# chinokikiss/GSV-TTS-Lite

Measured on AMD Instinct MI355X. Metric: semantic_tokens_per_sec_end_to_end (GPT AR incl. prefill + flow/Generator vocoder); RTF^-1 = value/25, higher is better.
Workload: dtype bf16; 1 GPU; configs[1]: v2Pro bs=1 greedy AR decode (250 tokens, kv 200->450) + flow/Generator vocoder (500 frames = 10 s audio) per GPU per step, hipGraph on; parallelism=replicas x1, ge broadcast once per speaker (0 tensor broadcasts in this run)

## Files before the change

### gsv-tts-lite_amd/csrc/gsv_abi.hip

```cpp
#include <hip/hip_runtime.h>

#include <algorithm>
#include <cmath>
#include <cstddef>
#include <cstdlib>
#include <cstring>
#include <cstdint>
#include <map>
#include <mutex>
#include <type_traits>
#include <unordered_map>
#include <utility>
#include <vector>

namespace gsv_arena {
struct Arena {
    std::vector<std::pair<char*, size_t>> blocks;
    size_t used = 0;
    size_t count = 0;
    std::unordered_map<void*, size_t> live;
    std::multimap<size_t, void*> freed;
};
static std::mutex g_mu;
static std::vector<std::pair<std::pair<char*, size_t>, Arena*>> g_all;
static thread_local Arena* g_cur = nullptr;
static hipError_t amalloc(void** p, size_t n) {
    if (!g_cur) return hipMalloc(p, n);
    static const size_t align = getenv("GSV_ARENA_ALIGN") ? (size_t)atol(getenv("GSV_ARENA_ALIGN")) : 65536;
    static const size_t skew = getenv("GSV_ARENA_SKEW") ? (size_t)atol(getenv("GSV_ARENA_SKEW")) : 0;
    constexpr size_t kBlock = (size_t)256 << 20;
    Arena& a = *g_cur;
    bool reuse = false;
    {
        std::lock_guard<std::mutex> lk(g_mu);
        auto it = a.freed.lower_bound(n);
        if (it != a.freed.end() && it->first <= n + std::max<size_t>(n / 4, align)) {
            *p = it->second;
            a.live[*p] = it->first;
            a.freed.erase(it);
            reuse = true;
        }
    }
    if (reuse) {
        return hipDeviceSynchronize();
    }
    const size_t sk = (a.count * skew) % align;
    size_t start = (a.used + align - 1) / align * align + sk;
    if (a.blocks.empty() || start + n > a.blocks.back().second) {
        const size_t sz = std::max(n + align, kBlock);
        char* base = nullptr;
        const hipError_t e = hipMalloc(&base, sz);
        if (e != hipSuccess) return e;
        a.blocks.emplace_back(base, sz);
        a.used = 0;
        start = sk;
        std::lock_guard<std::mutex> lk(g_mu);
        g_all.push_back({{base, sz}, &a});
    }
    *p = a.blocks.back().first + start;
    a.used = start + n;
    a.count++;
    std::lock_guard<std::mutex> lk(g_mu);
    a.live[*p] = n;
    return hipSuccess;
}
static hipError_t afree(void* p) {
    {
        std::lock_guard<std::mutex> lk(g_mu);
        for (auto& b : g_all)
            if ((char*)p >= b.first.first && (char*)p < b.first.first + b.first.second) {
                Arena& a = *b.second;
                auto it = a.live.find(p);
                if (it != a.live.end()) {
                    a.freed.emplace(it->second, p);
                    a.live.erase(it);
                }
                return hipSuccess;
            }
    }
    return hipFree(p);
}
static void release(Arena& a) {
    std::lock_guard<std::mutex> lk(g_mu);
    for (auto& b : a.blocks) {
        (void)hipFree(b.first);
        g_all.erase(std::remove_if(g_all.begin(), g_all.end(), [&](const std::pair<std::pair<char*, size_t>, Arena*>& e) { return e.first == b; }),
                    g_all.end());
    }
    a.blocks.clear();
    a.live.clear();
    a.freed.clear();
    a.used = 0;
}
struct Scope {
    Arena* prev;
    explicit Scope(Arena* a) : prev(g_cur) { g_cur = a; }
    ~Scope() { g_cur = prev; }
};
}
#define GSV_DEV_ALLOC_ARENA 1

#include "abi_common.h"
#include "t2s_decode.h"
#include "t2s_decode_multi.h"
#include "t2s_batch.h"
#include "t2s_small.h"

namespace {
thread_local std::string g_err;
}

int gsv::abi_fail(int code, const char* fmt, ...) {
    char buf[512];
    va_list ap;
    va_start(ap, fmt);
    vsnprintf(buf, sizeof(buf), fmt, ap);
    va_end(ap);
    g_err = buf;
    return code;
}

struct T2SLayer {
    void *wqkv_p = nullptr, *wo_p = nullptr, *w1 = nullptr, *w2_p = nullptr;
    void* w2_p64 = nullptr;
    float *bqkv_p = nullptr, *bo = nullptr, *b1 = nullptr, *b2 = nullptr, *ln1g = nullptr, *ln1b = nullptr,
          *ln2g = nullptr, *ln2b = nullptr;
    PackedConv g_qkv, g_out, g_w1, g_w2;
    void *p8_qkv = nullptr, *p8_w1 = nullptr, *p8_w2 = nullptr;
    void *p16_qkv = nullptr, *p16_out = nullptr, *p16_w1 = nullptr, *p16_w2 = nullptr;
    void *f8_qkv = nullptr, *f8_w1 = nullptr, *f8_w2 = nullptr;
    float *s_qkv = nullptr, *s_w1 = nullptr, *s_w2 = nullptr;
    unsigned have = 0;
};

struct T2SStateX : gsv_t2s_state {
    int32_t* eos_host = nullptr;
    u32x4* tab = nullptr;
};
static_assert(sizeof(gsv_t2s_slot_sampling) == sizeof(u32x4) * kSlotSamplingWords, "the token kernel reads an entry as two 16-byte words");
inline u32x4* tab_of(const gsv_t2s_state& s) { return static_cast<const T2SStateX&>(s).tab; }
inline int32_t* eos_host_of(const gsv_t2s_state& s) { return static_cast<const T2SStateX&>(s).eos_host; }

struct T2SBound {
    T2SStateX st;
    hipGraphExec_t graph = nullptr;
    hipGraphExec_t graph_ft = nullptr;
    static constexpr int kMaxWin = 8;
    hipGraphExec_t wgraph[2][kMaxWin + 1] = {};
    int64_t *sg_kv = nullptr, *sg_x = nullptr;
    int32_t *sg_step = nullptr, *sg_eos = nullptr;
    float *sg_logits = nullptr, *sg_hidden = nullptr;
    TokPart* sg_tok = nullptr;
};

void t2s_drop_graphs(T2SBound& b) {
    if (b.graph) { (void)hipGraphExecDestroy(b.graph); b.graph = nullptr; }
    if (b.graph_ft) { (void)hipGraphExecDestroy(b.graph_ft); b.graph_ft = nullptr; }
    for (auto& row : b.wgraph)
        for (hipGraphExec_t& g : row)
            if (g) { (void)hipGraphExecDestroy(g); g = nullptr; }
}

void t2s_free_staging(T2SBound& b) {
    for (void* p : {(void*)b.sg_kv, (void*)b.sg_x, (void*)b.sg_step, (void*)b.sg_eos, (void*)b.sg_logits, (void*)b.sg_hidden, (void*)b.sg_tok})
        if (p) (void)gsv_dev_free(p);
    b.sg_kv = b.sg_x = nullptr; b.sg_step = b.sg_eos = nullptr; b.sg_logits = b.sg_hidden = nullptr; b.sg_tok = nullptr;
}

struct gsv_t2s {
    gsv_t2s_config cfg;
    std::vector<T2SLayer> layers;
    void* predict = nullptr;
    float *emb_audio = nullptr, *emb_text = nullptr, *pe_audio = nullptr, *pe_text = nullptr;
    PackedConv g_bert;
    unsigned have_io = 0;
    bool finalized = false;
    bool fp8 = false;
    int batched_min = 0;
    int nt_from_layer = 0x7fffffff;
    std::map<int, T2SBound> bound;
    int scratch_b = 0;
    float *xcur = nullptr, *xbuf = nullptr, *x1buf = nullptr, *ypart = nullptr, *zpart = nullptr;
    TokPart* tokpart = nullptr;
    hipStream_t cap_stream = nullptr;
    unsigned long long* dbg = nullptr;
    gsv_arena::Arena arena;
    bool use_arena = true;
};
#define GSV_ARENA_SCOPE(h) gsv_arena::Scope arena_scope_((h)->use_arena ? &(h)->arena : nullptr)

namespace {

int t2s_pack_fp8(const float* data, int cout, int cin, void** frag, float** scale, hipStream_t st) {
    const int mtiles = cdiv(cout, 32);
    if (!*scale) HIPCHK(gsv_dev_malloc(scale, sizeof(float) * mtiles * 32));
    if (!*frag) HIPCHK(gsv_dev_malloc(frag, (size_t)mtiles * (cin / 32) * 64 * 16));
    HIPCHK(hipMemsetAsync(*scale, 0, sizeof(float) * mtiles * 32, st));
    hipLaunchKernelGGL(fp8_row_scale_kernel, dim3(cdiv(cout, 4)), dim3(256), 0, st, data, cin, *scale, cout);
    hipLaunchKernelGGL(fp8_pack_kernel, dim3(1024), dim3(256), 0, st, data, (const float*)*scale, (uint32_t*)*frag, cout, cin, mtiles);
    HIPCHK(hipGetLastError());
    return GSV_OK;
}

int t2s_pack16_f8(void** dst, const float* data, const float* scale, int N, int K, hipStream_t st) {
    if (!*dst) HIPCHK(gsv_dev_malloc(dst, (size_t)N * K));
    hipLaunchKernelGGL(pack16_f8_kernel, dim3(1024), dim3(256), 0, st, data, scale, (uint32_t*)*dst, N, K);
    HIPCHK(hipGetLastError());
    return GSV_OK;
}

template <typename WT>
int t2s_pack16(void** dst, const float* data, int N, int K, hipStream_t st) {
    if (sizeof(WT) != 2) return GSV_OK;
    if (!*dst) HIPCHK(gsv_dev_malloc(dst, sizeof(bf16_t) * (size_t)N * K));
    hipLaunchKernelGGL(pack16_kernel, dim3(1024), dim3(256), 0, st, data, (bf16_t*)*dst, N, K);
    HIPCHK(hipGetLastError());
    return GSV_OK;
}

template <typename WT>
int t2s_load_layer_tensor(gsv_t2s* h, int l, const std::string& key, const float* data, int64_t numel, hipStream_t st) {
    T2SLayer& L = h->layers[l];
    auto want = [&](int64_t n) { return numel == n ? GSV_OK : fail(GSV_ERR_ARG, "layer %d %s: numel %lld, expected %lld", l, key.c_str(), (long long)numel, (long long)n); };
    auto copy_f32 = [&](float** dst, int64_t n, unsigned bit) -> int {
        if (int rc = want(n)) return rc;
        if (!*dst) HIPCHK(gsv_dev_malloc(dst, sizeof(float) * n));
        HIPCHK(hipMemcpyAsync(*dst, data, sizeof(float) * n, hipMemcpyDeviceToDevice, st));
        L.have |= bit;
        return GSV_OK;
    };
    if (key == "qkv.weight") {
        if (int rc = want(3LL * kD * kD)) return rc;
        if (!L.wqkv_p) HIPCHK(gsv_dev_malloc(&L.wqkv_p, sizeof(WT) * 3 * kD * kD));
        hipLaunchKernelGGL((pack_qkv_panel_kernel<WT>), dim3(1024), dim3(256), 0, st, data, (WT*)L.wqkv_p);
        float* keep = L.g_qkv.bias; L.g_qkv.bias = nullptr;
        free_conv(L.g_qkv);
        if (int rc = pack_conv<WT>(L.g_qkv, data, 3 * kD, kD, 1, kD, 1, 0, 1, 0, 0, nullptr, 1.f, st)) return rc;
        L.g_qkv.bias = keep;
        if (h->fp8) if (int rc = t2s_pack_fp8(data, 3 * kD, kD, &L.f8_qkv, &L.s_qkv, st)) return rc;
        if (h->fp8) if (int rc = t2s_pack16_f8(&L.p8_qkv, data, L.s_qkv, 3 * kD, kD, st)) return rc;
        if (int rc = t2s_pack16<WT>(&L.p16_qkv, data, 3 * kD, kD, st)) return rc;
        L.have |= 1u << 0;
    } else if (key == "qkv.bias") {
        if (int rc = want(3 * kD)) return rc;
        if (!L.bqkv_p) HIPCHK(gsv_dev_malloc(&L.bqkv_p, sizeof(float) * 3 * kD));
        hipLaunchKernelGGL(pack_qkv_bias_kernel, dim3(6), dim3(256), 0, st, data, L.bqkv_p);
        if (!L.g_qkv.bias) HIPCHK(gsv_dev_malloc(&L.g_qkv.bias, sizeof(float) * 3 * kD));
        HIPCHK(hipMemcpyAsync(L.g_qkv.bias, data, sizeof(float) * 3 * kD, hipMemcpyDeviceToDevice, st));
        L.have |= 1u << 1;
    } else if (key == "out_proj.weight") {
        if (int rc = want((int64_t)kD * kD)) return rc;
        if (!L.wo_p) HIPCHK(gsv_dev_malloc(&L.wo_p, sizeof(WT) * kD * kD));
        hipLaunchKernelGGL((pack_col_panel_kernel<WT>), dim3(512), dim3(256), 0, st, data, (WT*)L.wo_p, kH, kDh);
        free_conv(L.g_out);
        if (int rc = pack_conv<WT>(L.g_out, data, kD, kD, 1, kD, 1, 0, 1, 0, 0, nullptr, 1.f, st)) return rc;
        if (int rc = t2s_pack16<WT>(&L.p16_out, data, kD, kD, st)) return rc;
        L.have |= 1u << 2;
    } else if (key == "out_proj.bias") {
        if (int rc = copy_f32(&L.bo, kD, 1u << 3)) return rc;
    } else if (key == "mlp.0.weight") {
        if (int rc = want((int64_t)kF * kD)) return rc;
        if (!L.w1) HIPCHK(gsv_dev_malloc(&L.w1, sizeof(WT) * kF * kD));
        hipLaunchKernelGGL((convert_kernel<WT>), dim3(1024), dim3(256), 0, st, data, (WT*)L.w1, (size_t)kF * kD);
        free_conv(L.g_w1);
        if (int rc = pack_conv<WT>(L.g_w1, data, kF, kD, 1, kD, 1, 0, 1, 0, 0, nullptr, 1.f, st)) return rc;
        if (h->fp8) if (int rc = t2s_pack_fp8(data, kF, kD, &L.f8_w1, &L.s_w1, st)) return rc;
        if (h->fp8) if (int rc = t2s_pack16_f8(&L.p8_w1, data, L.s_w1, kF, kD, st)) return rc;
        if (int rc = t2s_pack16<WT>(&L.p16_w1, data, kF, kD, st)) return rc;
        L.have |= 1u << 4;
    } else if (key == "mlp.0.bias") {
        if (int rc = copy_f32(&L.b1, kF, 1u << 5)) return rc;
    } else if (key == "mlp.2.weight") {
        if (int rc = want((int64_t)kD * kF)) return rc;
        if (!L.w2_p) HIPCHK(gsv_dev_malloc(&L.w2_p, sizeof(WT) * kD * kF));
        hipLaunchKernelGGL((pack_col_panel_kernel<WT>), dim3(1024), dim3(256), 0, st, data, (WT*)L.w2_p, kNJ, kFJ);
        {
            if (!L.w2_p64) HIPCHK(gsv_dev_malloc(&L.w2_p64, sizeof(WT) * kD * kF));
            hipLaunchKernelGGL((pack_col_panel_kernel<WT>), dim3(1024), dim3(256), 0, st, data, (WT*)L.w2_p64, kNJFine, kF / kNJFine);
        }
        free_conv(L.g_w2);
        if (int rc = pack_conv<WT>(L.g_w2, data, kD, kF, 1, kF, 1, 0, 1, 0, 0, nullptr, 1.f, st)) return rc;
        if (h->fp8) if (int rc = t2s_pack_fp8(data, kD, kF, &L.f8_w2, &L.s_w2, st)) return rc;
        if (h->fp8) if (int rc = t2s_pack16_f8(&L.p8_w2, data, L.s_w2, kD, kF, st)) return rc;
        if (int rc = t2s_pack16<WT>(&L.p16_w2, data, kD, kF, st)) return rc;
        L.have |= 1u << 6;
    } else if (key == "mlp.2.bias") {
        if (int rc = copy_f32(&L.b2, kD, 1u << 7)) return rc;
    } else if (key == "norm1.weight") {
        if (int rc = copy_f32(&L.ln1g, kD, 1u << 8)) return rc;
    } else if (key == "norm1.bias") {
        if (int rc = copy_f32(&L.ln1b, kD, 1u << 9)) return rc;
    } else if (key == "norm2.weight") {
        if (int rc = copy_f32(&L.ln2g, kD, 1u << 10)) return rc;
    } else if (key == "norm2.bias") {
        if (int rc = copy_f32(&L.ln2b, kD, 1u << 11)) return rc;
    } else {
        return fail(GSV_ERR_ARG, "unknown layer tensor '%s'", key.c_str());
    }
    HIPCHK(hipGetLastError());
    return GSV_OK;
}

template <typename WT>
int t2s_load_io_tensor(gsv_t2s* h, const std::string& name, const float* data, int64_t numel, hipStream_t st) {
    const gsv_t2s_config& c = h->cfg;
    auto copy_f32 = [&](float** dst, int64_t n, unsigned bit) -> int {
        if (numel != n) return fail(GSV_ERR_ARG, "%s: numel %lld, expected %lld", name.c_str(), (long long)numel, (long long)n);
        if (!*dst) HIPCHK(gsv_dev_malloc(dst, sizeof(float) * n));
        HIPCHK(hipMemcpyAsync(*dst, data, sizeof(float) * n, hipMemcpyDeviceToDevice, st));
        h->have_io |= bit;
        return GSV_OK;
    };
    if (name == "ar_predict_layer.weight") {
        if (numel != (int64_t)c.vocab * kD) return fail(GSV_ERR_ARG, "%s: bad numel", name.c_str());
        if (!h->predict) HIPCHK(gsv_dev_malloc(&h->predict, sizeof(WT) * c.vocab * kD));
        hipLaunchKernelGGL((convert_kernel<WT>), dim3(512), dim3(256), 0, st, data, (WT*)h->predict, (size_t)c.vocab * kD);
        h->have_io |= 1u << 0;
    } else if (name == "ar_audio_embedding.word_embeddings.weight") {
        return copy_f32(&h->emb_audio, (int64_t)c.vocab * kD, 1u << 1);
    } else if (name == "ar_text_embedding.word_embeddings.weight") {
        return copy_f32(&h->emb_text, (int64_t)c.n_phoneme * kD, 1u << 2);
    } else if (name == "ar_audio_position.pe_scaled") {
        return copy_f32(&h->pe_audio, (int64_t)c.n_pos * kD, 1u << 3);
    } else if (name == "ar_text_position.pe_scaled") {
        return copy_f32(&h->pe_text, (int64_t)c.n_pos * kD, 1u << 4);
    } else if (name == "bert_proj.weight") {
        if (numel != (int64_t)kD * 1024) return fail(GSV_ERR_ARG, "%s: bad numel", name.c_str());
        float* keep = h->g_bert.bias; h->g_bert.bias = nullptr;
        free_conv(h->g_bert);
        if (int rc = pack_conv<WT>(h->g_bert, data, kD, 1024, 1, 1024, 1, 0, 1, 0, 0, nullptr, 1.f, st)) return rc;
        h->g_bert.bias = keep;
        h->have_io |= 1u << 5;
    } else if (name == "bert_proj.bias") {
        return copy_f32(&h->g_bert.bias, kD, 1u << 6);
    } else if (name == "ar_text_position.alpha" || name == "ar_audio_position.alpha") {
        return GSV_OK;
    } else {
        return fail(GSV_ERR_ARG, "unknown tensor '%s'", name.c_str());
    }
    HIPCHK(hipGetLastError());
    return GSV_OK;
}

int t2s_ensure_scratch(gsv_t2s* h, int B) {
    if (B <= h->scratch_b) return GSV_OK;
    for (void* p : {(void*)h->xcur, (void*)h->xbuf, (void*)h->x1buf, (void*)h->ypart, (void*)h->zpart, (void*)h->tokpart})
        if (p) (void)gsv_dev_free(p);
    HIPCHK(gsv_dev_malloc(&h->xcur, sizeof(float) * B * kD));
    HIPCHK(gsv_dev_malloc(&h->xbuf, sizeof(float) * B * kD));
    HIPCHK(gsv_dev_malloc(&h->x1buf, sizeof(float) * B * kD));
    HIPCHK(gsv_dev_malloc(&h->ypart, sizeof(float) * B * kH * kD));
    HIPCHK(gsv_dev_malloc(&h->zpart, sizeof(float) * B * kNJFine * kD));
    HIPCHK(gsv_dev_malloc(&h->tokpart, sizeof(TokPart) * B * kNP));
    HIPCHK(hipMemset(h->tokpart, 0, sizeof(TokPart) * B * kNP));
    h->scratch_b = B;
    for (auto& kv : h->bound) t2s_drop_graphs(kv.second);
    return GSV_OK;
}

template <typename WT>
void t2s_launch_attn(gsv_t2s* h, const gsv_t2s_state& s, int l, const float* xsrc, hipStream_t st, bool fused_token = false) {
    const int B = s.batch, T = s.max_kv;
    const size_t lds = 0;
    const size_t layer_elems = (size_t)B * kH * T * kDh;
    T2SLayer& L = h->layers[l];
    AttnArgs<WT> a;
    a.xdirect = xsrc;
    a.zpart = (const typename Geo<WT>::PT*)h->zpart;
    a.b2 = l ? h->layers[l - 1].b2 : nullptr;
    a.x1 = h->x1buf;
    a.ln2g = l ? h->layers[l - 1].ln2g : nullptr;
    a.ln2b = l ? h->layers[l - 1].ln2b : nullptr;
    a.xout = h->xbuf;
    a.wqkv = (const WT*)L.wqkv_p; a.bqkv = L.bqkv_p; a.wo = (const WT*)L.wo_p;
    a.kc = (WT*)s.k_cache + (size_t)l * layer_elems;
    a.vc = (WT*)s.v_cache + (size_t)l * layer_elems;
    a.kv_len = s.kv_len; a.T = T; a.ypart = (typename Geo<WT>::PT*)h->ypart; a.dbg = (l == h->cfg.n_layer - 1) ? h->dbg : nullptr;
    if (l == 0 && fused_token) {
        StepTok& k = a.tk;
        k.tokpart = h->tokpart; k.tok_override = s.tok_override; k.ctl = s.ctl; k.x_len = s.x_len; k.pre_tokens = s.pre_tokens;
        k.seen = s.seen; k.step = s.step; k.eos_at = s.eos_at; k.emb = h->emb_audio; k.pe = h->pe_audio; k.eos_host = eos_host_of(s);
        k.V = h->cfg.vocab; k.eos = h->cfg.eos; k.n_pos = h->cfg.n_pos;
    }
    auto with_mode = [&](auto launch) {
        if (l == 0 && fused_token) launch(std::integral_constant<int, 2>{});
        else if (l == 0) launch(std::integral_constant<int, 0>{});
        else launch(std::integral_constant<int, 1>{});
    };
    if (B > 16) {
        const size_t ml = sizeof(float) * attn_multi_lds_floats<2>();
        with_mode([&](auto mode) { hipLaunchKernelGGL((t2s_attn_multi_kernel<WT, decltype(mode)::value, 2>), dim3(kH, cdiv(B, 2)), dim3(kNT), ml, st, a, B); });
        return;
    }
    auto single = [&](auto nj, auto nt, auto ntkv) {
        with_mode([&](auto mode) {
            constexpr int MODE = decltype(mode)::value;
            constexpr int NJ = MODE == 1 ? decltype(nj)::value : kNJ;
            constexpr bool NT = MODE == 1 && decltype(nt)::value;
            hipLaunchKernelGGL((t2s_attn_kernel<WT, MODE, NJ, NT, decltype(ntkv)::value>), dim3(kH, B), dim3(kNT), lds, st, a);
        });
    };
    using Coarse = std::integral_constant<int, kNJ>;
    using Fine = std::integral_constant<int, kNJFine>;
    using NtF32 = std::bool_constant<sizeof(WT) == 4>;
    const bool fine = ffn_slices(B) == kNJFine;
    static const int kvnt_b = getenv("GSV_SEQ_KV_NT_MIN_B") ? atoi(getenv("GSV_SEQ_KV_NT_MIN_B")) : 4;
    if (sizeof(WT) == 2 && B >= kvnt_b) {
        if (fine) single(Fine{}, std::false_type{}, std::true_type{});
        else single(Coarse{}, std::false_type{}, std::true_type{});
        return;
    }
    const bool nt = sizeof(WT) == 4 && l >= h->nt_from_layer;
    if (fine && nt) single(Fine{}, NtF32{}, std::false_type{});
    else if (fine) single(Fine{}, std::false_type{}, std::false_type{});
    else if (nt) single(Coarse{}, NtF32{}, std::false_type{});
    else single(Coarse{}, std::false_type{}, std::false_type{});
}

template <typename WT>
void t2s_launch_ffn(gsv_t2s* h, const gsv_t2s_state& s, int l, hipStream_t st) {
    T2SLayer& L = h->layers[l];
    FfnArgs<WT> f;
    f.ypart = (const typename Geo<WT>::PT*)h->ypart; f.bo = L.bo; f.x = h->xbuf; f.ln1g = L.ln1g; f.ln1b = L.ln1b; f.x1out = h->x1buf;
    f.w1 = (const WT*)L.w1; f.b1 = L.b1; f.w2p = (const WT*)L.w2_p; f.zpart = (typename Geo<WT>::PT*)h->zpart; f.dbg = (l == h->cfg.n_layer - 1) ? h->dbg : nullptr;
    const int B = s.batch;
    static const int ffn_single_max_b = getenv("GSV_FFN_SINGLE_MAX_B") ? atoi(getenv("GSV_FFN_SINGLE_MAX_B")) : 8;
    if (B > ffn_single_max_b) {
        hipLaunchKernelGGL((t2s_ffn_multi_kernel<WT, 2>), dim3(kNJ, cdiv(B, 2)), dim3(kNT), sizeof(float) * ffn_multi_lds_floats<2>(), st, f, B);
        return;
    }
    auto single = [&](auto nj) {
        constexpr int NJ = decltype(nj)::value;
        if (sizeof(WT) == 4 && l >= h->nt_from_layer) hipLaunchKernelGGL((t2s_ffn_kernel<WT, NJ, sizeof(WT) == 4>), dim3(NJ, B), dim3(kNT), 0, st, f);
        else hipLaunchKernelGGL((t2s_ffn_kernel<WT, NJ>), dim3(NJ, B), dim3(kNT), 0, st, f);
    };
    if (ffn_slices(B) == kNJFine) {
        f.w2p = (const WT*)L.w2_p64;
        single(std::integral_constant<int, kNJFine>{});
    } else {
        single(std::integral_constant<int, kNJ>{});
    }
}

template <typename WT>
int t2s_multi_lds_attr() {
    const int la = (int)(sizeof(float) * attn_multi_lds_floats<2>());
    HIPCHK(hipFuncSetAttribute((const void*)t2s_attn_multi_kernel<WT, 0, 2>, hipFuncAttributeMaxDynamicSharedMemorySize, la));
    HIPCHK(hipFuncSetAttribute((const void*)t2s_attn_multi_kernel<WT, 1, 2>, hipFuncAttributeMaxDynamicSharedMemorySize, la));
    HIPCHK(hipFuncSetAttribute((const void*)t2s_attn_multi_kernel<WT, 2, 2>, hipFuncAttributeMaxDynamicSharedMemorySize, la));
    HIPCHK(hipFuncSetAttribute((const void*)t2s_ffn_multi_kernel<WT, 2>, hipFuncAttributeMaxDynamicSharedMemorySize, (int)(sizeof(float) * ffn_multi_lds_floats<2>())));
    return GSV_OK;
}

template <typename WT>
int t2s_layers(gsv_t2s* h, const gsv_t2s_state& s, const float* xsrc, hipStream_t st, bool fused_token = false) {
    for (int l = 0; l < h->cfg.n_layer; ++l) {
        t2s_launch_attn<WT>(h, s, l, xsrc, st, fused_token);
        t2s_launch_ffn<WT>(h, s, l, st);
    }
    HIPCHK(hipGetLastError());
    return GSV_OK;
}

template <typename WT>
int t2s_logits(gsv_t2s* h, const gsv_t2s_state& s, int mode, const float* hdirect, int slot0, int nrows, int vlimit,
               int bump, hipStream_t st, const int32_t* slots = nullptr, const T2SBound* staged = nullptr) {
    const T2SLayer& L = h->layers.back();
    LogitsArgs<WT> a;
    a.hdirect = hdirect; a.zpart = (const typename Geo<WT>::PT*)h->zpart; a.b2 = L.b2; a.x1 = h->x1buf; a.ln2g = L.ln2g; a.ln2b = L.ln2b;
    a.wp = (const WT*)h->predict; a.V = h->cfg.vocab; a.eos = h->cfg.eos; a.vlimit = vlimit; a.slot0 = slot0; a.slots = slots;
    a.step = s.step; a.ctl = s.ctl; a.fctl = s.fctl; a.seen = s.seen; a.logits = s.logits; a.hidden = s.hidden;
    a.tokpart = h->tokpart; a.kv_len = s.kv_len; a.bump = bump;
    if (staged) { a.step = staged->sg_step; a.logits = staged->sg_logits; a.hidden = staged->sg_hidden; a.tokpart = staged->sg_tok; a.kv_len = staged->sg_kv; }
    a.tab = tab_of(s);
    auto launch = [&](auto tab) {
        constexpr bool TAB = decltype(tab)::value;
        if (mode == 0) hipLaunchKernelGGL((t2s_logits_kernel<WT, 0, kNJ, TAB>), dim3(kNP, nrows), dim3(kNT), 0, st, a);
        else if (ffn_slices(s.batch) == kNJFine) hipLaunchKernelGGL((t2s_logits_kernel<WT, 1, kNJFine, TAB>), dim3(kNP, nrows), dim3(kNT), 0, st, a);
        else hipLaunchKernelGGL((t2s_logits_kernel<WT, 1, kNJ, TAB>), dim3(kNP, nrows), dim3(kNT), 0, st, a);
    };
    if (a.tab) launch(std::true_type{});
    else launch(std::false_type{});
    HIPCHK(hipGetLastError());
    return GSV_OK;
}

int t2s_token(gsv_t2s* h, const gsv_t2s_state& s, int advance, hipStream_t st) {
    TokenArgs a;
    a.tokpart = h->tokpart; a.tok_override = s.tok_override; a.ctl = s.ctl; a.kv_len = s.kv_len; a.x_len = s.x_len;
    a.pre_tokens = s.pre_tokens; a.seen = s.seen; a.step = s.step; a.eos_at = s.eos_at; a.eos_host = eos_host_of(s); a.emb = h->emb_audio;
    a.pe = h->pe_audio; a.xcur = h->xcur; a.T = s.max_kv; a.V = h->cfg.vocab; a.eos = h->cfg.eos; a.n_pos = h->cfg.n_pos;
    a.advance = advance;
    a.logits = s.logits; a.fctl = s.fctl; a.tab = tab_of(s);
    if (a.tab) hipLaunchKernelGGL(t2s_token_kernel<true>, dim3(s.batch), dim3(256), 0, st, a);
    else hipLaunchKernelGGL(t2s_token_kernel<false>, dim3(s.batch), dim3(256), 0, st, a);
    HIPCHK(hipGetLastError());
    return GSV_OK;
}

constexpr int kBatchedMinDefault = 17;
constexpr int kWideMinM = 3072;
constexpr size_t kPrefillLdsMax = 160 * 1024;
constexpr int kNtFromLayerF32 = 9;

struct ChainBufs {
    float *qkv, *attn, *y1, *y2, *x1;
    void* hid;
};

template <typename AttnFn>
int t2s_gemm_chain(gsv_t2s* h, int M, float* x0, const ChainBufs& c, bool f8, AttnFn attn_launch, hipStream_t st, bool prompt = false) {
    const int rtiles = cdiv(M, 32);
    const int cpb = !prompt ? 1 : (rtiles < 40 ? 2 : (rtiles < 100 ? 4 : 8));
    auto run = [&](auto kern, int nthreads, BGemmArgs ba, int which = -1) {
        int cb = cpb;
        if (prompt && which >= 0) {
            if (rtiles <= 20 && (which == 1 || which == 3)) cb = 1;
            if (rtiles > 20 && rtiles < 40 && (which == 0 || which == 2)) cb = 4;
        }
        ba.cpb = cb;
        hipLaunchKernelGGL(kern, dim3(rtiles, cdiv(ba.mtiles, cb)), dim3(nthreads), 0, st, ba);
    };
    static const int small_max = getenv("GSV_SMALL_MAX_M") ? atoi(getenv("GSV_SMALL_MAX_M")) : kSmallMaxM;
    const bool small = !prompt && M <= small_max && h->layers[0].p16_qkv != nullptr && (!f8 || h->layers[0].p8_qkv != nullptr);
    const int rt16 = cdiv(M, 16);
    const bool nwv4 = M > 48;
    static const int wide_min = getenv("GSV_WIDE_MIN_M") ? atoi(getenv("GSV_WIDE_MIN_M")) : kWideMinM;
    const bool wide = prompt && !f8 && M >= wide_min;
    auto run_wide = [&](auto kern, bool w2, BGemmArgs ba) -> int {
        const int rgroups = cdiv(M, 32 * kWideRT), cgroups = cdiv(ba.mtiles, 4 * kWideTPW);
        int gpb = 1;
        if (!w2) {
            double best = 1e30;
            for (int g = 1; g <= cgroups; ++g) {
                if (cgroups % g) continue;
                const double cost = (double)cdiv(rgroups * (cgroups / g), 256) * (1.0 + g);
                if (cost < best - 1e-9) { best = cost; gpb = g; }
            }
        }
        ba.cpb = gpb * 4 * kWideTPW;
        hipLaunchKernelGGL(kern, dim3(rgroups, cgroups / gpb), dim3(256), kWideLds, st, ba);
        return GSV_OK;
    };
    for (int l = 0; l < h->cfg.n_layer; ++l) {
        T2SLayer& L = h->layers[l];
        if (wide) {
            {
                BGemmArgs g{};
                g.M = M; g.ldx = kD; g.W = (const uint4*)L.g_qkv.w; g.mtiles = 3 * kD / 32; g.cout = 3 * kD; g.bias = L.g_qkv.bias; g.Y = c.qkv; g.ldy = 3 * kD;
                if (l == 0) {
                    g.X = x0;
                    if (int rc = run_wide(bgemm_wide_kernel<PRO_NONE, float, bf16_t>, false, g)) return rc;
                } else {
                    g.X = c.y2; g.lng = h->layers[l - 1].ln2g; g.lnb = h->layers[l - 1].ln2b; g.xout = x0;
                    if (int rc = run_wide(bgemm_wide_kernel<PRO_LN, float, bf16_t>, false, g)) return rc;
                }
            }
            attn_launch(l);
            {
                BGemmArgs g{};
                g.M = M; g.X = c.attn; g.ldx = kD; g.W = (const uint4*)L.g_out.w; g.mtiles = kD / 32; g.cout = kD; g.bias = L.bo;
                g.res = x0; g.ldres = kD; g.Y = c.y1; g.ldy = kD;
                if (int rc = run_wide(bgemm_wide_kernel<PRO_NONE, bf16_t, float>, false, g)) return rc;
            }
            {
                BGemmArgs g{};
                g.M = M; g.X = c.y1; g.ldx = kD; g.lng = L.ln1g; g.lnb = L.ln1b; g.xout = c.x1;
                g.W = (const uint4*)L.g_w1.w; g.mtiles = kF / 32; g.cout = kF; g.bias = L.b1; g.relu = 1; g.Y = c.hid; g.ldy = kF;
                if (int rc = run_wide(bgemm_wide_kernel<PRO_LN, float, bf16_t>, false, g)) return rc;
            }
            {
                BGemmArgs g{};
                g.M = M; g.X = c.hid; g.ldx = kF; g.W = (const uint4*)L.g_w2.w; g.mtiles = kD / 32; g.cout = kD;
                g.bias = L.b2; g.res = c.x1; g.ldres = kD; g.Y = c.y2; g.ldy = kD;
                if (int rc = run_wide(bgemm_wide_kernel<PRO_NONE, bf16_t, float>, true, g)) return rc;
            }
            continue;
        }
        if (small) {
            {
                SGemmArgs g{};
                g.M = M; g.W = (const uint4*)(f8 ? L.p8_qkv : L.p16_qkv); g.wscale = L.s_qkv; g.bias = L.g_qkv.bias; g.Y = c.qkv; g.ldy = 3 * kD;
                const dim3 grid(rt16, 3 * kD / 32);
                if (l == 0) {
                    g.X = x0;
                    if (f8) hipLaunchKernelGGL((sgemm_kernel<PRO_NONE, float, 2, true>), grid, dim3(128), 0, st, g);
                    else hipLaunchKernelGGL((sgemm_kernel<PRO_NONE, float, 2>), grid, dim3(128), 0, st, g);
                } else {
                    g.X = c.y2; g.lng = h->layers[l - 1].ln2g; g.lnb = h->layers[l - 1].ln2b; g.xout = x0;
                    const dim3 grid4(rt16, 3 * kD / 64);
                    if (f8 && nwv4) hipLaunchKernelGGL((sgemm_kernel<PRO_LN, float, 4, true>), grid4, dim3(256), 0, st, g);
                    else if (f8) hipLaunchKernelGGL((sgemm_kernel<PRO_LN, float, 2, true>), grid, dim3(128), 0, st, g);
                    else if (nwv4) hipLaunchKernelGGL((sgemm_kernel<PRO_LN, float, 4>), grid4, dim3(256), 0, st, g);
                    else hipLaunchKernelGGL((sgemm_kernel<PRO_LN, float, 2>), grid, dim3(128), 0, st, g);
                }
            }
            attn_launch(l);
            {
                SGemmArgs g{};
                g.M = M; g.X = c.attn; g.W = (const uint4*)L.p16_out; g.bias = L.bo; g.res = x0; g.Y = c.y1; g.ldy = kD;
                hipLaunchKernelGGL((sgemm_kernel<PRO_NONE, float, 2>), dim3(rt16, kD / 32), dim3(128), 0, st, g);
            }
            {
                SGemmArgs g{};
                g.M = M; g.X = c.y1; g.lng = L.ln1g; g.lnb = L.ln1b; g.xout = c.x1; g.W = (const uint4*)(f8 ? L.p8_w1 : L.p16_w1); g.wscale = L.s_w1;
                g.bias = L.b1; g.relu = 1; g.Y = c.hid; g.ldy = kF;
                if (f8 && nwv4) hipLaunchKernelGGL((sgemm_kernel<PRO_LN, fp8_t, 4, true>), dim3(rt16, kF / 64), dim3(256), 0, st, g);
                else if (f8) hipLaunchKernelGGL((sgemm_kernel<PRO_LN, fp8_t, 2, true>), dim3(rt16, kF / 32), dim3(128), 0, st, g);
                else if (nwv4) hipLaunchKernelGGL((sgemm_kernel<PRO_LN, bf16_t, 4>), dim3(rt16, kF / 64), dim3(256), 0, st, g);
                else hipLaunchKernelGGL((sgemm_kernel<PRO_LN, bf16_t, 2>), dim3(rt16, kF / 32), dim3(128), 0, st, g);
            }
            {
                SGemmArgs g{};
                g.M = M; g.X = c.hid; g.W = (const uint4*)(f8 ? L.p8_w2 : L.p16_w2); g.wscale = L.s_w2; g.bias = L.b2; g.res = c.x1; g.Y = c.y2; g.ldy = kD;
                if (f8) hipLaunchKernelGGL(sgemm_k_kernel<true>, dim3(rt16, kD / 16), dim3(256), 0, st, g);
                else hipLaunchKernelGGL(sgemm_k_kernel<false>, dim3(rt16, kD / 16), dim3(256), 0, st, g);
            }
            continue;
        }
        {
            BGemmArgs g{};
            g.M = M; g.ldx = kD; g.W = (const uint4*)(f8 ? L.f8_qkv : L.g_qkv.w); g.wscale = L.s_qkv; g.mtiles = 3 * kD / 32; g.cout = 3 * kD;
            g.bias = L.g_qkv.bias; g.Y = c.qkv; g.ldy = 3 * kD;
            if (l == 0) {
                g.X = x0;
                if (f8) run(bgemm_kernel<PRO_NONE, float, float, 4, true>, 256, g);
                else if (prompt) run(bgemm_kernel<PRO_NONE, float, bf16_t, 4, false, true>, 256, g, 0);
                else run(bgemm_kernel<PRO_NONE, float, float, 4, false, true>, 256, g);
            } else {
                g.X = c.y2; g.lng = h->layers[l - 1].ln2g; g.lnb = h->layers[l - 1].ln2b; g.xout = x0;
                if (f8) run(bgemm_kernel<PRO_LN, float, float, 4, true>, 256, g);
                else if (prompt) run(bgemm_kernel<PRO_LN, float, bf16_t, 4, false, true>, 256, g, 0);
                else run(bgemm_kernel<PRO_LN, float, float, 4, false, true>, 256, g);
            }
        }
        attn_launch(l);
        {
            BGemmArgs g{};
            g.M = M; g.X = c.attn; g.ldx = kD; g.W = (const uint4*)L.g_out.w; g.mtiles = kD / 32; g.cout = kD; g.bias = L.bo;
            g.res = x0; g.ldres = kD; g.Y = c.y1; g.ldy = kD;
            if (prompt) run(bgemm_kernel<PRO_NONE, bf16_t, float, 4, false>, 256, g, 1);
            else run(bgemm_kernel<PRO_NONE, float, float, 4, false, true>, 256, g);
        }
        {
            BGemmArgs g{};
            g.M = M; g.X = c.y1; g.ldx = kD; g.lng = L.ln1g; g.lnb = L.ln1b; g.xout = c.x1;
            g.W = (const uint4*)(f8 ? L.f8_w1 : L.g_w1.w); g.wscale = L.s_w1; g.mtiles = kF / 32; g.cout = kF; g.bias = L.b1; g.relu = 1;
            g.Y = c.hid; g.ldy = kF;
            if (f8) run(bgemm_kernel<PRO_LN, float, fp8_t, 4, true>, 256, g);
            else run(bgemm_kernel<PRO_LN, float, bf16_t, 4, false, true>, 256, g, 2);
        }
        {
            BGemmArgs g{};
            g.M = M; g.X = c.hid; g.ldx = kF; g.W = (const uint4*)(f8 ? L.f8_w2 : L.g_w2.w); g.wscale = L.s_w2; g.mtiles = kD / 32; g.cout = kD;
            g.bias = L.b2; g.res = c.x1; g.ldres = kD; g.Y = c.y2; g.ldy = kD;
            if (f8) run(bgemm_kernel<PRO_NONE, fp8_t, float, 16, true>, 1024, g);
            else run(bgemm_kernel<PRO_NONE, bf16_t, float, 16, false>, 1024, g, 3);
        }
    }
    HIPCHK(hipGetLastError());
    return GSV_OK;
}

template <typename WT>
int t2s_batched_layers(gsv_t2s* h, const gsv_t2s_state& s, hipStream_t st) {
    const int B = s.batch, T = s.max_kv;
    ChainBufs c;
    c.qkv = h->ypart;
    c.attn = c.qkv + (size_t)B * 3 * kD;
    c.y1 = c.attn + (size_t)B * kD;
    c.y2 = c.y1 + (size_t)B * kD;
    c.x1 = h->x1buf;
    c.hid = h->zpart;
    const size_t layer_elems = (size_t)B * kH * T * kDh;
    auto attn = [&](int l) {
        BatchAttnArgs<WT> ba;
        ba.qkv = c.qkv; ba.kc = (WT*)s.k_cache + (size_t)l * layer_elems; ba.vc = (WT*)s.v_cache + (size_t)l * layer_elems;
        ba.kv_len = s.kv_len; ba.T = T; ba.out = c.attn; ba.dbg = (l == h->cfg.n_layer - 1) ? h->dbg : nullptr;
        if (T <= 256) hipLaunchKernelGGL((t2s_batch_attn2_kernel<4, true>), dim3(kH, B), dim3(256), 0, st, ba);
        else if (T <= 512) hipLaunchKernelGGL((t2s_batch_attn2_kernel<8, true>), dim3(kH, B), dim3(256), 0, st, ba);
        else hipLaunchKernelGGL((t2s_batch_attn2_kernel<16, true>), dim3(kH, B), dim3(256), 0, st, ba);
    };
    if (int rc = t2s_gemm_chain(h, B, h->xcur, c, h->fp8, attn, st)) return rc;
    const T2SLayer& LL = h->layers.back();
    hipLaunchKernelGGL(ln_rows_kernel, dim3(cdiv(B, 4)), dim3(256), 0, st, (const float*)c.y2, (const float*)LL.ln2g, (const float*)LL.ln2b, h->xbuf, B);
    HIPCHK(hipGetLastError());
    return GSV_OK;
}

template <typename WT>
int t2s_step(gsv_t2s* h, const gsv_t2s_state& s, hipStream_t st, bool fused_token = false) {
    if (fused_token && !(sizeof(WT) == 2 && s.batch >= h->batched_min && s.max_kv <= 1024)) {
        if (int rc = t2s_layers<WT>(h, s, h->xcur, st, true)) return rc;
        return t2s_logits<WT>(h, s, 1, nullptr, 0, s.batch, h->cfg.vocab, 1, st);
    }
    if (int rc = t2s_token(h, s, 1, st)) return rc;
    if constexpr (sizeof(WT) == 2) {
        if (s.batch >= h->batched_min && s.max_kv <= 1024) {
            if (int rc = t2s_batched_layers<WT>(h, s, st)) return rc;
            return t2s_logits<WT>(h, s, 0, h->xbuf, 0, s.batch, h->cfg.vocab, 1, st);
        }
    }
    if (int rc = t2s_layers<WT>(h, s, h->xcur, st)) return rc;
    return t2s_logits<WT>(h, s, 1, nullptr, 0, s.batch, h->cfg.vocab, 1, st);
}

template <typename WT>
int t2s_prefill_impl(gsv_t2s* h, T2SBound& bd, int slot0, int nrows, int l_max, float* xy, const int64_t* x_lens,
                     const int64_t* y_lens, void* ws, size_t ws_bytes, hipStream_t st, const int32_t* slots = nullptr, bool staged = false) {
    const gsv_t2s_state& s = bd.st;
    const int M = nrows * l_max, T = s.max_kv;
    const size_t need = gsv_t2s_prefill_workspace(h, nrows, l_max);
    if (ws_bytes < need) return fail(GSV_ERR_ARG, "prefill workspace %zu < %zu", ws_bytes, need);
    float* qkv = (float*)ws;
    float* attn = qkv + (size_t)M * 3 * kD;
    float* ybuf = attn + (size_t)M * kD;
    float* fbuf = ybuf + (size_t)M * kD;
    float* hlast = fbuf + (size_t)M * kF;
    const size_t layer_elems = (size_t)s.batch * kH * T * kDh;
    const int qsplit = std::max(1, std::min(16, 256 / (kH * nrows)));
    const size_t lds = sizeof(float) * ((size_t)l_max * 33 + (size_t)l_max * 32 + 4 * (size_t)l_max + 128 + 8);
    const int nkt_max = cdiv(l_max, 32);
    const size_t lds_mfma = (size_t)nkt_max * 32 * 80 + 128 * 80 + (size_t)32 * (nkt_max * 64 + 16);
    if (sizeof(WT) == 2 ? lds_mfma > kPrefillLdsMax : lds > kPrefillLdsMax)
        return fail(GSV_ERR_ARG, "prefill: prompt of %d positions exceeds the LDS-staged attention limit of the %s mode (%d positions)",
                    l_max, sizeof(WT) == 2 ? "bf16" : "fp32", sizeof(WT) == 2 ? 1056 : 591);
    if constexpr (sizeof(WT) == 2) {
        ChainBufs c;
        c.qkv = qkv; c.attn = attn; c.y1 = ybuf; c.y2 = fbuf; c.x1 = fbuf + (size_t)M * kD; c.hid = fbuf + (size_t)2 * M * kD;
        auto attn_launch = [&](int l) {
            PrefillAttnMfmaArgs pm;
            pm.qkv = (const bf16_t*)qkv; pm.x_lens = x_lens; pm.y_lens = y_lens;
            pm.kc = (bf16_t*)s.k_cache + (size_t)l * layer_elems; pm.vc = (bf16_t*)s.v_cache + (size_t)l * layer_elems;
            pm.T = T; pm.slot0 = slot0; pm.slots = slots; pm.l_max = l_max; pm.out = (bf16_t*)attn;
            hipLaunchKernelGGL(t2s_prefill_attn_mfma_kernel, dim3(kH, nrows, cdiv(l_max, 128)), dim3(256), lds_mfma, st, pm);
        };
        if (int rc = t2s_gemm_chain(h, M, xy, c, false, attn_launch, st, true)) return rc;
        const T2SLayer& LL = h->layers.back();
        hipLaunchKernelGGL(ln_rows_kernel, dim3(cdiv(M, 4)), dim3(256), 0, st, (const float*)c.y2, (const float*)LL.ln2g, (const float*)LL.ln2b, xy, M);
        HIPCHK(hipGetLastError());
    } else {
        for (int l = 0; l < h->cfg.n_layer; ++l) {
            T2SLayer& L = h->layers[l];
            Epi e0; e0.fixed_order = true;
            if (int rc = run_conv<float, WT, float>(L.g_qkv, xy, kD, M, qkv, 3 * kD, M, e0, st)) return rc;
            PrefillAttnArgs<WT> pa;
            pa.qkv = qkv; pa.x_lens = x_lens; pa.y_lens = y_lens;
            pa.kc = (WT*)s.k_cache + (size_t)l * layer_elems; pa.vc = (WT*)s.v_cache + (size_t)l * layer_elems;
            pa.T = T; pa.slot0 = slot0; pa.slots = slots; pa.l_max = l_max; pa.qsplit = qsplit; pa.out = attn;
            {
                hipLaunchKernelGGL((t2s_prefill_attn_kernel<WT>), dim3(kH, nrows, qsplit), dim3(256), lds, st, pa);
            }
            Epi e1; e1.res = xy; e1.ld_res = kD; e1.fixed_order = true;
            PackedConv go = L.g_out; go.bias = L.bo;
            if (int rc = run_conv<float, WT, float>(go, attn, kD, M, ybuf, kD, M, e1, st)) return rc;
            hipLaunchKernelGGL(ln_rows_kernel, dim3(cdiv(M, 4)), dim3(256), 0, st, ybuf, L.ln1g, L.ln1b, xy, M);
            Epi e2; e2.act = ACT_RELU; e2.fixed_order = true;
            PackedConv g1 = L.g_w1; g1.bias = L.b1;
            if (int rc = run_conv<float, WT, float>(g1, xy, kD, M, fbuf, kF, M, e2, st)) return rc;
            Epi e3; e3.res = xy; e3.ld_res = kD; e3.fixed_order = true;
            PackedConv g2 = L.g_w2; g2.bias = L.b2;
            if (int rc = run_conv<float, WT, float>(g2, fbuf, kF, M, ybuf, kD, M, e3, st)) return rc;
            hipLaunchKernelGGL(ln_rows_kernel, dim3(cdiv(M, 4)), dim3(256), 0, st, ybuf, L.ln2g, L.ln2b, xy, M);
        }
    }
    PrefillFinishArgs fa;
    fa.hidden = xy; fa.x_lens = x_lens; fa.y_lens = y_lens; fa.hlast = hlast; fa.kv_len = s.kv_len; fa.x_len = s.x_len;
    fa.step = s.step; fa.eos_at = s.eos_at; fa.eos_host = bd.st.eos_host; fa.slot0 = slot0; fa.slots = slots; fa.l_max = l_max;
    if (staged) { fa.kv_len = bd.sg_kv; fa.x_len = bd.sg_x; fa.step = bd.sg_step; fa.eos_at = bd.sg_eos; fa.eos_host = nullptr; }
    hipLaunchKernelGGL(t2s_prefill_finish_kernel, dim3(nrows), dim3(128), 0, st, fa);
    HIPCHK(hipGetLastError());
    return t2s_logits<WT>(h, s, 0, hlast, slot0, nrows, h->cfg.vocab - 1, 0, st, slots, staged ? &bd : nullptr);
}

struct CommitArgs {
    const int32_t* slots;
    const int64_t *sg_kv, *sg_x; const int32_t *sg_step, *sg_eos; const float *sg_logits, *sg_hidden; const TokPart* sg_tok;
    int64_t *kv_len, *x_len; int32_t *step, *eos_at, *eos_host; float *logits, *hidden; TokPart* tokpart;
    int V;
};
__global__ __launch_bounds__(256) void t2s_commit_kernel(CommitArgs a) {
    const int s = a.slots[blockIdx.x], tid = threadIdx.x;
    for (int v = tid; v < a.V; v += 256) a.logits[(size_t)s * a.V + v] = a.sg_logits[(size_t)s * a.V + v];
    for (int c = tid; c < kD; c += 256) a.hidden[(size_t)s * kD + c] = a.sg_hidden[(size_t)s * kD + c];
    if (tid < kNP) a.tokpart[(size_t)s * kNP + tid] = a.sg_tok[(size_t)s * kNP + tid];
    if (tid == 0) { a.kv_len[s] = a.sg_kv[s]; a.x_len[s] = a.sg_x[s]; a.step[s] = a.sg_step[s]; a.eos_at[s] = a.sg_eos[s]; eos_publish(a.eos_host, s, a.sg_eos[s]); }
}


constexpr int kAdoptMax = 64;
struct AdoptArgs {
    short dst[kAdoptMax], src[kAdoptMax];
    long long ovr[kAdoptMax];
    const unsigned char *ks, *vs;
    unsigned char *kd, *vd;
    int Bs, Ts, Bd, Td, esz;
    const int64_t *sg_kv, *sg_x; const int32_t *sg_step, *sg_eos; const float *sg_logits, *sg_hidden; const TokPart* sg_tok;
    int64_t *kv_len, *x_len, *tok_override; int32_t *step, *eos_at, *eos_host; float *logits, *hidden; TokPart* tokpart;
    const unsigned char* s_seen; unsigned char* d_seen;
    int V;
};
__global__ __launch_bounds__(256) void t2s_adopt_kv_kernel(AdoptArgs a) {
    const int lh = blockIdx.x, r = blockIdx.y, l = lh / kH, hd = lh % kH;
    const int ss = a.src[r], ds = a.dst[r];
    long long kv = a.sg_kv[ss];
    kv = kv < 0 ? 0 : (kv > a.Ts ? a.Ts : kv);
    kv = kv > a.Td ? a.Td : kv;
    const size_t n16 = (size_t)kv * kDh * a.esz / 16;
    const size_t so = ((((size_t)l * a.Bs + ss) * kH + hd) * a.Ts) * kDh * a.esz;
    const size_t d0 = ((((size_t)l * a.Bd + ds) * kH + hd) * a.Td) * kDh * a.esz;
    const uint4* sp = reinterpret_cast<const uint4*>((blockIdx.z ? a.vs : a.ks) + so);
    uint4* dp = reinterpret_cast<uint4*>((blockIdx.z ? a.vd : a.kd) + d0);
    for (size_t i = threadIdx.x; i < n16; i += 256) dp[i] = sp[i];
}
__global__ __launch_bounds__(256) void t2s_adopt_state_kernel(AdoptArgs a) {
    const int ss = a.src[blockIdx.x], s = a.dst[blockIdx.x], tid = threadIdx.x;
    for (int v = tid; v < a.V; v += 256) { a.logits[(size_t)s * a.V + v] = a.sg_logits[(size_t)ss * a.V + v]; a.d_seen[(size_t)s * a.V + v] = a.s_seen[(size_t)ss * a.V + v]; }
    for (int c = tid; c < kD; c += 256) a.hidden[(size_t)s * kD + c] = a.sg_hidden[(size_t)ss * kD + c];
    if (tid < kNP) a.tokpart[(size_t)s * kNP + tid] = a.sg_tok[(size_t)ss * kNP + tid];
    if (tid == 0) {
        a.kv_len[s] = a.sg_kv[ss]; a.x_len[s] = a.sg_x[ss]; a.step[s] = a.sg_step[ss]; a.eos_at[s] = a.sg_eos[ss];
        eos_publish(a.eos_host, s, a.sg_eos[ss]);
        if (a.ovr[blockIdx.x] >= 0) a.tok_override[s] = a.ovr[blockIdx.x];
    }
}

struct MoveArgs {
    short dst[kAdoptMax], src[kAdoptMax];
    const unsigned char *ks, *vs; unsigned char *kd, *vd;
    int Bs, Ts, Bd, Td, esz, V, n;
    const int64_t *s_kv, *s_x, *s_pre, *s_ovr; const int32_t *s_step, *s_eos; const float *s_logits, *s_hidden; const unsigned char* s_seen;
    int64_t *d_kv, *d_x, *d_pre, *d_ovr; int32_t *d_step, *d_eos, *d_eos_host; float *d_logits, *d_hidden; unsigned char* d_seen;
    TokPart* tokpart;
    const u32x4* s_tab; u32x4* d_tab;
};
__global__ __launch_bounds__(256) void t2s_move_kv_kernel(MoveArgs a) {
    const int lh = blockIdx.x, r = blockIdx.y, l = lh / kH, hd = lh % kH;
    const int ss = a.src[r], ds = a.dst[r];
    long long kv = a.s_kv[ss];
    kv = kv < 0 ? 0 : (kv > a.Ts ? a.Ts : kv);
    kv = kv > a.Td ? a.Td : kv;
    const size_t n16 = (size_t)kv * kDh * a.esz / 16;
    const size_t so = ((((size_t)l * a.Bs + ss) * kH + hd) * a.Ts) * kDh * a.esz;
    const size_t d0 = ((((size_t)l * a.Bd + ds) * kH + hd) * a.Td) * kDh * a.esz;
    const uint4* sp = reinterpret_cast<const uint4*>((blockIdx.z ? a.vs : a.ks) + so);
    uint4* dp = reinterpret_cast<uint4*>((blockIdx.z ? a.vd : a.kd) + d0);
    for (size_t i = threadIdx.x; i < n16; i += 256) dp[i] = sp[i];
}
__global__ __launch_bounds__(256) void t2s_move_state_kernel(MoveArgs a) {
    const int tid = threadIdx.x;
    if (blockIdx.x == a.n) {
        __shared__ TokPart tp[kAdoptMax * kNP];
        for (int i = tid; i < a.n * kNP; i += 256) tp[i] = a.tokpart[(size_t)a.src[i / kNP] * kNP + i % kNP];
        __syncthreads();
        for (int i = tid; i < a.n * kNP; i += 256) a.tokpart[(size_t)a.dst[i / kNP] * kNP + i % kNP] = tp[i];
        return;
    }
    const int ss = a.src[blockIdx.x], s = a.dst[blockIdx.x];
    for (int v = tid; v < a.V; v += 256) { a.d_logits[(size_t)s * a.V + v] = a.s_logits[(size_t)ss * a.V + v]; a.d_seen[(size_t)s * a.V + v] = a.s_seen[(size_t)ss * a.V + v]; }
    for (int c = tid; c < kD; c += 256) a.d_hidden[(size_t)s * kD + c] = a.s_hidden[(size_t)ss * kD + c];
    const int np = (a.Ts < a.Td ? a.Ts : a.Td) + 1;
    for (int t = tid; t < np; t += 256) a.d_pre[(size_t)s * (a.Td + 1) + t] = a.s_pre[(size_t)ss * (a.Ts + 1) + t];
    if (tid == 0) {
        a.d_kv[s] = a.s_kv[ss]; a.d_x[s] = a.s_x[ss]; a.d_step[s] = a.s_step[ss]; a.d_eos[s] = a.s_eos[ss]; a.d_ovr[s] = a.s_ovr[ss];
        eos_publish(a.d_eos_host, s, a.s_eos[ss]);
    }
    if (a.s_tab != nullptr && tid < kSlotSamplingWords) a.d_tab[kSlotSamplingWords * s + tid] = a.s_tab[kSlotSamplingWords * ss + tid];
}

struct PutSamplingArgs {
    short slot[kAdoptMax];
    u32x4 e[kAdoptMax][kSlotSamplingWords];
    u32x4* tab;
};
__global__ __launch_bounds__(64) void t2s_put_sampling_kernel(PutSamplingArgs a) {
    const int r = blockIdx.x, tid = threadIdx.x;
    if (tid < kSlotSamplingWords) a.tab[kSlotSamplingWords * a.slot[r] + tid] = a.e[r][tid];
}

struct SeedSeenArgs {
    short slot[kAdoptMax];
    int off[kAdoptMax + 1];
    const int64_t* tokens;
    unsigned char* seen;
    int V;
};
__global__ __launch_bounds__(256) void t2s_seed_seen_kernel(SeedSeenArgs a) {
    const int r = blockIdx.x, tid = threadIdx.x;
    unsigned char* row = a.seen + (size_t)a.slot[r] * a.V;
    for (int v = tid; v < a.V; v += 256) row[v] = 0;
    __syncthreads();
    for (int i = a.off[r] + tid; i < a.off[r + 1]; i += 256) {
        const int64_t t = a.tokens[i];
        if (t >= 0 && t < a.V) row[t] = 1;
    }
}

}

template <typename WT>
static int t2s_time_impl(gsv_t2s* h, T2SBound* b, int iters, float* out_ms, hipStream_t st) {
    struct Guard {
        hipEvent_t e0 = nullptr, e1 = nullptr;
        hipGraphExec_t exec = nullptr;
        ~Guard() {
            if (exec) (void)hipGraphExecDestroy(exec);
            if (e0) (void)hipEventDestroy(e0);
            if (e1) (void)hipEventDestroy(e1);
        }
    } gd;
    HIPCHK(hipEventCreate(&gd.e0));
    HIPCHK(hipEventCreate(&gd.e1));
    const int NL = h->cfg.n_layer;
    for (int cls = 0; cls < 4; ++cls) {
        hipGraph_t g = nullptr;
        HIPCHK(hipStreamSynchronize(st));
        HIPCHK(hipStreamBeginCapture(h->cap_stream, hipStreamCaptureModeThreadLocal));
        int rc = GSV_OK;
        for (int l = 0; l < NL && !rc; ++l) {
            if (cls == 0) t2s_launch_attn<WT>(h, b->st, l, h->xcur, h->cap_stream);
            if (cls == 1) t2s_launch_ffn<WT>(h, b->st, l, h->cap_stream);
            if (cls == 2) rc = t2s_logits<WT>(h, b->st, 1, nullptr, 0, b->st.batch, h->cfg.vocab, 0, h->cap_stream);
            if (cls == 3) rc = t2s_token(h, b->st, 0, h->cap_stream);
        }
        hipError_t e = hipStreamEndCapture(h->cap_stream, &g);
        if (rc) { if (g) (void)hipGraphDestroy(g); return rc; }
        if (e != hipSuccess) return fail(GSV_ERR_HIP, "hipStreamEndCapture: %s", hipGetErrorString(e));
        e = hipGraphInstantiate(&gd.exec, g, nullptr, nullptr, 0);
        (void)hipGraphDestroy(g);
        if (e != hipSuccess) { gd.exec = nullptr; return fail(GSV_ERR_HIP, "hipGraphInstantiate: %s", hipGetErrorString(e)); }
        HIPCHK(hipGraphLaunch(gd.exec, st));
        HIPCHK(hipEventRecord(gd.e0, st));
        for (int it = 0; it < iters; ++it) HIPCHK(hipGraphLaunch(gd.exec, st));
        HIPCHK(hipEventRecord(gd.e1, st));
        HIPCHK(hipEventSynchronize(gd.e1));
        float ms = 0.f;
        HIPCHK(hipEventElapsedTime(&ms, gd.e0, gd.e1));
        out_ms[cls] = ms / (float)(iters * NL);
        (void)hipGraphExecDestroy(gd.exec);
        gd.exec = nullptr;
    }
    return GSV_OK;
}

extern "C" {

int gsv_version(void) { return 1; }
const char* gsv_last_error(void) { return g_err.c_str(); }

int gsv_t2s_create(const gsv_t2s_config* cfg, gsv_t2s** out) {
    if (!cfg || !out) return fail(GSV_ERR_ARG, "null argument");
    if (cfg->hidden != kD || cfg->n_head != kH)
        return fail(GSV_ERR_ARG, "unsupported GPT shape: hidden %d heads %d (kernels are specialised for 512/16)", cfg->hidden, cfg->n_head);
    if (cfg->vocab < 2 || cfg->vocab > kNP * 128 || cfg->n_layer < 1 || cfg->n_pos < 1)
        return fail(GSV_ERR_ARG, "unsupported vocab/n_layer/n_pos");
    if (cfg->dtype != GSV_F32 && cfg->dtype != GSV_BF16 && cfg->dtype != GSV_FP8) return fail(GSV_ERR_ARG, "bad dtype");
    gsv_t2s* h = new gsv_t2s();
    h->cfg = *cfg;
    if (cfg->dtype == GSV_FP8) { h->fp8 = true; h->cfg.dtype = GSV_BF16; }
    h->batched_min = kBatchedMinDefault;
    if (const char* e = getenv("GSV_BATCHED_MIN")) h->batched_min = std::max(1, atoi(e));
    if (h->cfg.dtype == GSV_F32) h->nt_from_layer = kNtFromLayerF32;
    if (const char* e = getenv("GSV_NT_FROM_LAYER")) h->nt_from_layer = atoi(e);
    if (getenv("GSV_NO_ARENA")) h->use_arena = false;
    h->layers.resize(cfg->n_layer);
    if (hipStreamCreateWithFlags(&h->cap_stream, hipStreamNonBlocking) != hipSuccess) {
        delete h;
        return fail(GSV_ERR_HIP, "hipStreamCreate failed");
    }
    *out = h;
    return GSV_OK;
}

int gsv_t2s_destroy(gsv_t2s* h) {
    if (!h) return GSV_OK;
    (void)hipDeviceSynchronize();
    for (auto& kv : h->bound) {
        t2s_drop_graphs(kv.second);
        t2s_free_staging(kv.second);
    }
    for (T2SLayer& L : h->layers) {
        for (void* p : {L.wqkv_p, L.wo_p, L.w1, L.w2_p, L.w2_p64, L.p16_qkv, L.p16_out, L.p16_w1, L.p16_w2, L.p8_qkv, L.p8_w1, L.p8_w2, (void*)L.bqkv_p, (void*)L.bo, (void*)L.b1, (void*)L.b2,
                        (void*)L.ln1g, (void*)L.ln1b, (void*)L.ln2g, (void*)L.ln2b, L.f8_qkv, L.f8_w1, L.f8_w2,
                        (void*)L.s_qkv, (void*)L.s_w1, (void*)L.s_w2})
            if (p) (void)gsv_dev_free(p);
        free_conv(L.g_qkv); L.g_out.bias = nullptr; free_conv(L.g_out); L.g_w1.bias = nullptr; free_conv(L.g_w1);
        L.g_w2.bias = nullptr; free_conv(L.g_w2);
    }
    for (void* p : {h->predict, (void*)h->emb_audio, (void*)h->emb_text, (void*)h->pe_audio, (void*)h->pe_text,
                    (void*)h->xcur, (void*)h->xbuf, (void*)h->x1buf, (void*)h->ypart, (void*)h->zpart, (void*)h->tokpart})
        if (p) (void)gsv_dev_free(p);
    free_conv(h->g_bert);
    if (h->cap_stream) (void)hipStreamDestroy(h->cap_stream);
    gsv_arena::release(h->arena);
    delete h;
    return GSV_OK;
}

int gsv_t2s_load_tensor(gsv_t2s* h, const char* name, const float* data, int64_t numel, void* stream) {
    if (!h || !name || !data) return fail(GSV_ERR_ARG, "null argument");
    GSV_ARENA_SCOPE(h);
    std::string n(name);
    const std::string pre = "t2s_transformer.blocks.";
    h->finalized = false;
    if (n.compare(0, pre.size(), pre) == 0) {
        size_t dot = n.find('.', pre.size());
        if (dot == std::string::npos) return fail(GSV_ERR_ARG, "bad tensor name '%s'", name);
        int l = atoi(n.substr(pre.size(), dot - pre.size()).c_str());
        if (l < 0 || l >= h->cfg.n_layer) return fail(GSV_ERR_ARG, "layer index out of range in '%s'", name);
        std::string key = n.substr(dot + 1);
        return h->cfg.dtype == GSV_BF16 ? t2s_load_layer_tensor<bf16_t>(h, l, key, data, numel, S(stream))
                                        : t2s_load_layer_tensor<float>(h, l, key, data, numel, S(stream));
    }
    return h->cfg.dtype == GSV_BF16 ? t2s_load_io_tensor<bf16_t>(h, n, data, numel, S(stream))
                                    : t2s_load_io_tensor<float>(h, n, data, numel, S(stream));
}

int gsv_t2s_finalize(gsv_t2s* h, void* stream) {
    if (!h) return fail(GSV_ERR_ARG, "null handle");
    GSV_ARENA_SCOPE(h);
    for (int l = 0; l < h->cfg.n_layer; ++l)
        if (h->layers[l].have != 0xfffu) return fail(GSV_ERR_STATE, "layer %d incomplete (mask 0x%x)", l, h->layers[l].have);
    if (h->have_io != 0x7fu) return fail(GSV_ERR_STATE, "embedding/predict tensors incomplete (mask 0x%x)", h->have_io);
    if (h->cfg.dtype == GSV_BF16) {
        HIPCHK(hipFuncSetAttribute((const void*)t2s_prefill_attn_mfma_kernel, hipFuncAttributeMaxDynamicSharedMemorySize, (int)kPrefillLdsMax));
        HIPCHK(hipFuncSetAttribute((const void*)bgemm_wide_kernel<PRO_NONE, float, bf16_t>, hipFuncAttributeMaxDynamicSharedMemorySize, (int)kWideLds));
        HIPCHK(hipFuncSetAttribute((const void*)bgemm_wide_kernel<PRO_LN, float, bf16_t>, hipFuncAttributeMaxDynamicSharedMemorySize, (int)kWideLds));
        HIPCHK(hipFuncSetAttribute((const void*)bgemm_wide_kernel<PRO_NONE, bf16_t, float>, hipFuncAttributeMaxDynamicSharedMemorySize, (int)kWideLds));
        if (int rc = t2s_multi_lds_attr<bf16_t>()) return rc;
    } else {
        HIPCHK(hipFuncSetAttribute((const void*)t2s_prefill_attn_kernel<float>, hipFuncAttributeMaxDynamicSharedMemorySize, (int)kPrefillLdsMax));
        if (int rc = t2s_multi_lds_attr<float>()) return rc;
    }
    HIPCHK(hipStreamSynchronize(S(stream)));
    h->finalized = true;
    return GSV_OK;
}

int gsv_t2s_bind_state(gsv_t2s* h, const gsv_t2s_state* st) {
    if (!h || !st) return fail(GSV_ERR_ARG, "null argument");
    GSV_ARENA_SCOPE(h);
    if (st->batch < 1 || st->max_kv < 2) return fail(GSV_ERR_ARG, "bad batch/max_kv");
    if (!st->k_cache || !st->v_cache || !st->kv_len || !st->x_len || !st->pre_tokens || !st->seen || !st->step ||
        !st->eos_at || !st->logits || !st->hidden || !st->tok_override || !st->ctl || !st->fctl)
        return fail(GSV_ERR_ARG, "state has null pointers");
    if (int rc = t2s_ensure_scratch(h, st->batch)) return rc;
    T2SBound& b = h->bound[st->batch];
    t2s_drop_graphs(b);
    static_cast<gsv_t2s_state&>(b.st) = *st;
    b.st.eos_host = nullptr;
    b.st.tab = nullptr;
    t2s_free_staging(b);
    const size_t B = (size_t)st->batch;
    HIPCHK(gsv_dev_malloc(&b.sg_kv, 8 * B)); HIPCHK(gsv_dev_malloc(&b.sg_x, 8 * B));
    HIPCHK(gsv_dev_malloc(&b.sg_step, 4 * B)); HIPCHK(gsv_dev_malloc(&b.sg_eos, 4 * B));
    HIPCHK(gsv_dev_malloc(&b.sg_logits, sizeof(float) * B * h->cfg.vocab)); HIPCHK(gsv_dev_malloc(&b.sg_hidden, sizeof(float) * B * kD));
    HIPCHK(gsv_dev_malloc(&b.sg_tok, sizeof(TokPart) * B * kNP));
    HIPCHK(hipMemset(b.sg_step, 0, 4 * B));
    HIPCHK(hipMemset(b.sg_kv, 0, 8 * B)); HIPCHK(hipMemset(b.sg_x, 0, 8 * B));
    HIPCHK(hipMemset(b.sg_eos, 0xff, 4 * B));
    return GSV_OK;
}

int gsv_t2s_unbind_state(gsv_t2s* h, int batch) {
    if (!h) return fail(GSV_ERR_ARG, "null handle");
    GSV_ARENA_SCOPE(h);
    auto it = h->bound.find(batch);
    if (it == h->bound.end()) return GSV_OK;
    T2SBound& b = it->second;
    t2s_drop_graphs(b);
    t2s_free_staging(b);
    h->bound.erase(it);
    return GSV_OK;
}

static T2SBound* t2s_find(gsv_t2s* h, int batch) {
    auto it = h->bound.find(batch);
    return it == h->bound.end() ? nullptr : &it->second;
}

int gsv_t2s_embed_prompt(gsv_t2s* h, int nrows, int lx_max, int ly_max, int l_max, const int64_t* x_ids,
                         const int64_t* y_ids, const float* bert, const int64_t* x_lens, const int64_t* y_lens,
                         float* xy, float* scratch, void* stream) {
    if (!h || !h->finalized) return fail(GSV_ERR_STATE, "handle not finalized");
    if (nrows < 1 || lx_max < 1 || ly_max < 1 || l_max < 1 || l_max > h->cfg.n_pos) return fail(GSV_ERR_ARG, "bad sizes");
    const int M = nrows * lx_max;
    Epi e;
    e.fixed_order = true;
    int rc = h->cfg.dtype == GSV_BF16 ? run_conv<float, bf16_t, float>(h->g_bert, bert, 1024, M, scratch, kD, M, e, S(stream))
                                      : run_conv<float, float, float>(h->g_bert, bert, 1024, M, scratch, kD, M, e, S(stream));
    if (rc) return rc;
    EmbedArgs a;
    a.x_ids = x_ids; a.y_ids = y_ids; a.proj = scratch; a.x_lens = x_lens; a.y_lens = y_lens; a.emb_text = h->emb_text;
    a.emb_audio = h->emb_audio; a.pe_text = h->pe_text; a.pe_audio = h->pe_audio; a.xy = xy; a.lx_max = lx_max;
    a.ly_max = ly_max; a.l_max = l_max; a.n_phoneme = h->cfg.n_phoneme; a.V = h->cfg.vocab;
    hipLaunchKernelGGL(t2s_embed_kernel, dim3(l_max, nrows), dim3(128), 0, S(stream), a);
    HIPCHK(hipGetLastError());
    return GSV_OK;
}

size_t gsv_t2s_prefill_workspace(gsv_t2s* h, int nrows, int l_max) {
    (void)h;
    const size_t M = (size_t)nrows * l_max;
    return sizeof(float) * (M * (3 * kD + kD + kD + kF) + (size_t)nrows * kD) + 256;
}

int gsv_t2s_prefill(gsv_t2s* h, int batch, int slot0, int nrows, int l_max, float* xy, const int64_t* x_lens,
                    const int64_t* y_lens, void* workspace, size_t workspace_bytes, void* stream) {
    if (!h || !h->finalized) return fail(GSV_ERR_STATE, "handle not finalized");
    T2SBound* b = t2s_find(h, batch);
    if (!b) return fail(GSV_ERR_STATE, "no state bound for batch %d", batch);
    if (slot0 < 0 || nrows < 1 || slot0 + nrows > batch) return fail(GSV_ERR_ARG, "slot range out of bounds");
    if (l_max < 1 || l_max > b->st.max_kv) return fail(GSV_ERR_ARG, "prompt of %d positions does not fit the KV cache (%d)", l_max, b->st.max_kv);
    return h->cfg.dtype == GSV_BF16
               ? t2s_prefill_impl<bf16_t>(h, *b, slot0, nrows, l_max, xy, x_lens, y_lens, workspace, workspace_bytes, S(stream))
               : t2s_prefill_impl<float>(h, *b, slot0, nrows, l_max, xy, x_lens, y_lens, workspace, workspace_bytes, S(stream));
}

int gsv_t2s_prefill_slots(gsv_t2s* h, int batch, const int32_t* slots, int nrows, int l_max, float* xy, const int64_t* x_lens,
                          const int64_t* y_lens, void* workspace, size_t workspace_bytes, void* stream) {
    if (!h || !h->finalized) return fail(GSV_ERR_STATE, "handle not finalized");
    T2SBound* b = t2s_find(h, batch);
    if (!b) return fail(GSV_ERR_STATE, "no state bound for batch %d", batch);
    if (!slots || nrows < 1 || nrows > batch) return fail(GSV_ERR_ARG, "prefill_slots: need 1..batch rows and their slot list");
    if (l_max < 1 || l_max > b->st.max_kv) return fail(GSV_ERR_ARG, "prompt of %d positions does not fit the KV cache (%d)", l_max, b->st.max_kv);
    return h->cfg.dtype == GSV_BF16
               ? t2s_prefill_impl<bf16_t>(h, *b, 0, nrows, l_max, xy, x_lens, y_lens, workspace, workspace_bytes, S(stream), slots)
               : t2s_prefill_impl<float>(h, *b, 0, nrows, l_max, xy, x_lens, y_lens, workspace, workspace_bytes, S(stream), slots);
}

int gsv_t2s_prefill_slots_staged(gsv_t2s* h, int batch, const int32_t* slots, int nrows, int l_max, float* xy, const int64_t* x_lens,
                                 const int64_t* y_lens, void* workspace, size_t workspace_bytes, void* stream) {
    if (!h || !h->finalized) return fail(GSV_ERR_STATE, "handle not finalized");
    T2SBound* b = t2s_find(h, batch);
    if (!b) return fail(GSV_ERR_STATE, "no state bound for batch %d", batch);
    if (!slots || nrows < 1 || nrows > batch) return fail(GSV_ERR_ARG, "prefill_slots_staged: need 1..batch rows and their slot list");
    if (l_max < 1 || l_max > b->st.max_kv - 1) return fail(GSV_ERR_ARG, "prompt of %d positions does not fit beside the parking row of the KV cache (%d)", l_max, b->st.max_kv);
    return h->cfg.dtype == GSV_BF16
               ? t2s_prefill_impl<bf16_t>(h, *b, 0, nrows, l_max, xy, x_lens, y_lens, workspace, workspace_bytes, S(stream), slots, true)
               : t2s_prefill_impl<float>(h, *b, 0, nrows, l_max, xy, x_lens, y_lens, workspace, workspace_bytes, S(stream), slots, true);
}

int gsv_t2s_commit_slots(gsv_t2s* h, int batch, const int32_t* slots, int nrows, void* stream) {
    if (!h || !h->finalized) return fail(GSV_ERR_STATE, "handle not finalized");
    T2SBound* b = t2s_find(h, batch);
    if (!b) return fail(GSV_ERR_STATE, "no state bound for batch %d", batch);
    if (!slots || nrows < 1 || nrows > batch) return fail(GSV_ERR_ARG, "commit_slots: need 1..batch slots");
    CommitArgs a;
    a.slots = slots; a.sg_kv = b->sg_kv; a.sg_x = b->sg_x; a.sg_step = b->sg_step; a.sg_eos = b->sg_eos; a.sg_logits = b->sg_logits;
    a.sg_hidden = b->sg_hidden; a.sg_tok = b->sg_tok; a.kv_len = b->st.kv_len; a.x_len = b->st.x_len; a.step = b->st.step; a.eos_at = b->st.eos_at; a.eos_host = b->st.eos_host;
    a.logits = b->st.logits; a.hidden = b->st.hidden; a.tokpart = h->tokpart; a.V = h->cfg.vocab;
    hipLaunchKernelGGL(t2s_commit_kernel, dim3(nrows), dim3(256), 0, S(stream), a);
    HIPCHK(hipGetLastError());
    return GSV_OK;
}

int gsv_t2s_adopt_slots(gsv_t2s* h, int batch_dst, const int32_t* slots_dst, int batch_src, const int32_t* slots_src,
                        const int64_t* tok_override, int nrows, void* stream) {
    if (!h || !h->finalized) return fail(GSV_ERR_STATE, "handle not finalized");
    T2SBound* d = t2s_find(h, batch_dst);
    T2SBound* sb = t2s_find(h, batch_src);
    if (!d || !sb) return fail(GSV_ERR_STATE, "no state bound for batch %d", d ? batch_src : batch_dst);
    if (d == sb) return fail(GSV_ERR_ARG, "adopt_slots: source and destination are the same state");
    if (!slots_dst || !slots_src || nrows < 1 || nrows > batch_dst || nrows > batch_src) return fail(GSV_ERR_ARG, "adopt_slots: need 1..batch slot pairs (host arrays)");
    if (d->st.k_cache == sb->st.k_cache || d->st.v_cache == sb->st.v_cache) return fail(GSV_ERR_ARG, "adopt_slots: the two states share their KV cache");
    if (sb->st.max_kv > d->st.max_kv) return fail(GSV_ERR_ARG, "adopt_slots: the source cache (%d positions) is longer than the destination's (%d)", sb->st.max_kv, d->st.max_kv);
    for (int i = 0; i < nrows; ++i) {
        if (slots_dst[i] < 0 || slots_dst[i] >= batch_dst || slots_src[i] < 0 || slots_src[i] >= batch_src) return fail(GSV_ERR_ARG, "adopt_slots: slot out of range");
        for (int j = 0; j < i; ++j) if (slots_dst[j] == slots_dst[i]) return fail(GSV_ERR_ARG, "adopt_slots: destination slot %d listed twice", slots_dst[i]);
    }
    AdoptArgs a;
    a.ks = (const unsigned char*)sb->st.k_cache; a.vs = (const unsigned char*)sb->st.v_cache; a.kd = (unsigned char*)d->st.k_cache; a.vd = (unsigned char*)d->st.v_cache;
    a.Bs = batch_src; a.Ts = sb->st.max_kv; a.Bd = batch_dst; a.Td = d->st.max_kv; a.esz = h->cfg.dtype == GSV_F32 ? 4 : 2;
    a.sg_kv = sb->sg_kv; a.sg_x = sb->sg_x; a.sg_step = sb->sg_step; a.sg_eos = sb->sg_eos; a.sg_logits = sb->sg_logits; a.sg_hidden = sb->sg_hidden; a.sg_tok = sb->sg_tok;
    a.kv_len = d->st.kv_len; a.x_len = d->st.x_len; a.tok_override = d->st.tok_override; a.step = d->st.step; a.eos_at = d->st.eos_at; a.eos_host = d->st.eos_host;
    a.logits = d->st.logits; a.hidden = d->st.hidden; a.tokpart = h->tokpart; a.V = h->cfg.vocab;
    a.s_seen = (const unsigned char*)sb->st.seen; a.d_seen = (unsigned char*)d->st.seen;
    for (int r0 = 0; r0 < nrows; r0 += kAdoptMax) {
        const int n = std::min(kAdoptMax, nrows - r0);
        for (int i = 0; i < n; ++i) { a.dst[i] = (short)slots_dst[r0 + i]; a.src[i] = (short)slots_src[r0 + i]; a.ovr[i] = tok_override ? (long long)tok_override[r0 + i] : -1; }
        hipLaunchKernelGGL(t2s_adopt_kv_kernel, dim3(h->cfg.n_layer * kH, n, 2), dim3(256), 0, S(stream), a);
        hipLaunchKernelGGL(t2s_adopt_state_kernel, dim3(n), dim3(256), 0, S(stream), a);
    }
    HIPCHK(hipGetLastError());
    return GSV_OK;
}

int gsv_t2s_move_slots(gsv_t2s* h, int batch_dst, const int32_t* slots_dst, int batch_src, const int32_t* slots_src, int nrows, void* stream) {
    if (!h || !h->finalized) return fail(GSV_ERR_STATE, "handle not finalized");
    T2SBound* d = t2s_find(h, batch_dst);
    T2SBound* sb = t2s_find(h, batch_src);
    if (!d || !sb) return fail(GSV_ERR_STATE, "no state bound for batch %d", d ? batch_src : batch_dst);
    if (d == sb) return fail(GSV_ERR_ARG, "move_slots: source and destination are the same state");
    if (!slots_dst || !slots_src || nrows < 1 || nrows > batch_dst || nrows > batch_src || nrows > kAdoptMax)
        return fail(GSV_ERR_ARG, "move_slots: need 1..min(batch, %d) slot pairs (host arrays)", kAdoptMax);
    if (d->st.k_cache == sb->st.k_cache || d->st.v_cache == sb->st.v_cache) return fail(GSV_ERR_ARG, "move_slots: the two states share their KV cache");
    if (sb->st.max_kv > d->st.max_kv) return fail(GSV_ERR_ARG, "move_slots: the source cache (%d positions) is longer than the destination's (%d)", sb->st.max_kv, d->st.max_kv);
    for (int i = 0; i < nrows; ++i) {
        if (slots_dst[i] < 0 || slots_dst[i] >= batch_dst || slots_src[i] < 0 || slots_src[i] >= batch_src) return fail(GSV_ERR_ARG, "move_slots: slot out of range");
        for (int j = 0; j < i; ++j)
            if (slots_dst[j] == slots_dst[i] || slots_src[j] == slots_src[i]) return fail(GSV_ERR_ARG, "move_slots: slot listed twice");
    }
    if (sb->st.tab && !d->st.tab)
        return fail(GSV_ERR_ARG, "move_slots: batch %d has a per-slot sampling table and batch %d has none: the moved slots' parameters would be lost", batch_src, batch_dst);
    MoveArgs a;
    a.s_tab = d->st.tab ? sb->st.tab : nullptr; a.d_tab = d->st.tab;
    a.ks = (const unsigned char*)sb->st.k_cache; a.vs = (const unsigned char*)sb->st.v_cache; a.kd = (unsigned char*)d->st.k_cache; a.vd = (unsigned char*)d->st.v_cache;
    a.Bs = batch_src; a.Ts = sb->st.max_kv; a.Bd = batch_dst; a.Td = d->st.max_kv; a.esz = h->cfg.dtype == GSV_F32 ? 4 : 2; a.V = h->cfg.vocab; a.n = nrows;
    a.s_kv = sb->st.kv_len; a.s_x = sb->st.x_len; a.s_pre = sb->st.pre_tokens; a.s_ovr = sb->st.tok_override; a.s_step = sb->st.step; a.s_eos = sb->st.eos_at;
    a.s_logits = sb->st.logits; a.s_hidden = sb->st.hidden; a.s_seen = (const unsigned char*)sb->st.seen;
    a.d_kv = d->st.kv_len; a.d_x = d->st.x_len; a.d_pre = d->st.pre_tokens; a.d_ovr = d->st.tok_override; a.d_step = d->st.step; a.d_eos = d->st.eos_at; a.d_eos_host = d->st.eos_host;
    a.d_logits = d->st.logits; a.d_hidden = d->st.hidden; a.d_seen = (unsigned char*)d->st.seen; a.tokpart = h->tokpart;
    for (int i = 0; i < nrows; ++i) { a.dst[i] = (short)slots_dst[i]; a.src[i] = (short)slots_src[i]; }
    hipLaunchKernelGGL(t2s_move_kv_kernel, dim3(h->cfg.n_layer * kH, nrows, 2), dim3(256), 0, S(stream), a);
    hipLaunchKernelGGL(t2s_move_state_kernel, dim3(nrows + 1), dim3(256), 0, S(stream), a);
    HIPCHK(hipGetLastError());
    return GSV_OK;
}

int gsv_t2s_decode_hidden(gsv_t2s* h, int batch, const float* x, void* stream) {
    if (!h || !h->finalized) return fail(GSV_ERR_STATE, "handle not finalized");
    T2SBound* b = t2s_find(h, batch);
    if (!b) return fail(GSV_ERR_STATE, "no state bound for batch %d", batch);
    if (h->cfg.dtype == GSV_BF16 && batch >= h->batched_min && b->st.max_kv <= 1024) {
        HIPCHK(hipMemcpyAsync(h->xcur, x, sizeof(float) * (size_t)batch * kD, hipMemcpyDeviceToDevice, S(stream)));
        if (int rc = t2s_batched_layers<bf16_t>(h, b->st, S(stream))) return rc;
        return t2s_logits<bf16_t>(h, b->st, 0, h->xbuf, 0, batch, h->cfg.vocab, 1, S(stream));
    }
    int rc = h->cfg.dtype == GSV_BF16 ? t2s_layers<bf16_t>(h, b->st, x, S(stream)) : t2s_layers<float>(h, b->st, x, S(stream));
    if (rc) return rc;
    return h->cfg.dtype == GSV_BF16 ? t2s_logits<bf16_t>(h, b->st, 1, nullptr, 0, batch, h->cfg.vocab, 1, S(stream))
                                    : t2s_logits<float>(h, b->st, 1, nullptr, 0, batch, h->cfg.vocab, 1, S(stream));
}

int gsv_t2s_decode(gsv_t2s* h, int batch, int n_steps, int use_graph, void* stream) {
    if (!h || !h->finalized) return fail(GSV_ERR_STATE, "handle not finalized");
    T2SBound* b = t2s_find(h, batch);
    if (!b) return fail(GSV_ERR_STATE, "no state bound for batch %d", batch);
    const bool bf = h->cfg.dtype == GSV_BF16;
    const bool graph = (use_graph & 1) != 0, ft = (use_graph & GSV_STEP_FUSED_TOKEN) != 0;
    if (!graph) {
        for (int i = 0; i < n_steps; ++i)
            if (int rc = bf ? t2s_step<bf16_t>(h, b->st, S(stream), ft) : t2s_step<float>(h, b->st, S(stream), ft)) return rc;
        return GSV_OK;
    }
    auto graph_of = [&](int steps, hipGraphExec_t** out) -> int {
        hipGraphExec_t& exec = steps == 1 ? (ft ? b->graph_ft : b->graph) : b->wgraph[ft ? 1 : 0][steps];
        *out = &exec;
        if (exec) return GSV_OK;
        hipGraph_t g = nullptr;
        HIPCHK(hipStreamBeginCapture(h->cap_stream, hipStreamCaptureModeThreadLocal));
        int rc = GSV_OK;
        for (int i = 0; i < steps && !rc; ++i) rc = bf ? t2s_step<bf16_t>(h, b->st, h->cap_stream, ft) : t2s_step<float>(h, b->st, h->cap_stream, ft);
        hipError_t e = hipStreamEndCapture(h->cap_stream, &g);
        if (rc) { if (g) (void)hipGraphDestroy(g); return rc; }
        if (e != hipSuccess) return fail(GSV_ERR_HIP, "hipStreamEndCapture: %s", hipGetErrorString(e));
        e = hipGraphInstantiate(&exec, g, nullptr, nullptr, 0);
        (void)hipGraphDestroy(g);
        if (e != hipSuccess) return fail(GSV_ERR_HIP, "hipGraphInstantiate: %s", hipGetErrorString(e));
        return GSV_OK;
    };
    static const int win_max = getenv("GSV_STEP_WINDOW") ? std::max(1, std::min((int)T2SBound::kMaxWin, atoi(getenv("GSV_STEP_WINDOW")))) : 5;
    int left = n_steps;
    while (left > 0) {
        const int w = std::min(left, win_max);
        hipGraphExec_t* exec = nullptr;
        if (int rc = graph_of(w, &exec)) return rc;
        HIPCHK(hipGraphLaunch(*exec, S(stream)));
        left -= w;
    }
    return GSV_OK;
}

int gsv_t2s_time_kernels(gsv_t2s* h, int batch, int iters, float* out_ms, void* stream) {
    if (!h || !h->finalized || !out_ms || iters < 1) return fail(GSV_ERR_STATE, "bad call");
    T2SBound* b = t2s_find(h, batch);
    if (!b) return fail(GSV_ERR_STATE, "no state bound for batch %d", batch);
    return h->cfg.dtype == GSV_BF16 ? t2s_time_impl<bf16_t>(h, b, iters, out_ms, S(stream))
                                    : t2s_time_impl<float>(h, b, iters, out_ms, S(stream));
}

int gsv_t2s_set_eos_mirror(gsv_t2s* h, int batch, int32_t* host_mapped) {
    if (!h || !h->finalized) return fail(GSV_ERR_STATE, "handle not finalized");
    T2SBound* b = t2s_find(h, batch);
    if (!b) return fail(GSV_ERR_STATE, "no state bound for batch %d", batch);
    b->st.eos_host = host_mapped;
    t2s_drop_graphs(*b);
    return GSV_OK;
}

int gsv_t2s_set_slot_sampling(gsv_t2s* h, int batch, gsv_t2s_slot_sampling* table) {
    if (!h || !h->finalized) return fail(GSV_ERR_STATE, "handle not finalized");
    T2SBound* b = t2s_find(h, batch);
    if (!b) return fail(GSV_ERR_STATE, "no state bound for batch %d", batch);
    if ((uintptr_t)table % 16 != 0) return fail(GSV_ERR_ARG, "set_slot_sampling: the table must be 16-byte aligned");
    if (b->st.tab == (u32x4*)table) return GSV_OK;
    b->st.tab = (u32x4*)table;
    t2s_drop_graphs(*b);
    return GSV_OK;
}

int gsv_t2s_put_slot_sampling(gsv_t2s* h, int batch, const int32_t* slots, const gsv_t2s_slot_sampling* entries, int nrows, void* stream) {
    if (!h || !h->finalized) return fail(GSV_ERR_STATE, "handle not finalized");
    T2SBound* b = t2s_find(h, batch);
    if (!b) return fail(GSV_ERR_STATE, "no state bound for batch %d", batch);
    if (!b->st.tab) return fail(GSV_ERR_STATE, "put_slot_sampling: batch %d has no per-slot sampling table (gsv_t2s_set_slot_sampling)", batch);
    if (!slots || !entries || nrows < 1) return fail(GSV_ERR_ARG, "put_slot_sampling: need slots and entries (host arrays)");
    for (int i = 0; i < nrows; ++i) {
        if (slots[i] < 0 || slots[i] >= batch) return fail(GSV_ERR_ARG, "put_slot_sampling: slot %d out of range", (int)slots[i]);
        if (entries[i].sample_mode != 0 && entries[i].sample_mode != 2)
            return fail(GSV_ERR_ARG, "put_slot_sampling: entry %d has sample_mode %d (0 = greedy, 2 = device sampling)", i, (int)entries[i].sample_mode);
        if (!std::isfinite(entries[i].rep_penalty) || entries[i].rep_penalty < 0.f)
            return fail(GSV_ERR_ARG, "put_slot_sampling: entry %d has rep_penalty %g (0 = off, else a finite number > 0)", i, (double)entries[i].rep_penalty);
        if (entries[i].suppress_steps < 0)
            return fail(GSV_ERR_ARG, "put_slot_sampling: entry %d has suppress_steps %d (>= 0)", i, (int)entries[i].suppress_steps);
    }
    PutSamplingArgs a;
    a.tab = b->st.tab;
    for (int r0 = 0; r0 < nrows; r0 += kAdoptMax) {
        const int n = std::min(kAdoptMax, nrows - r0);
        for (int i = 0; i < n; ++i) { a.slot[i] = (short)slots[r0 + i]; memcpy(a.e[i], &entries[r0 + i], sizeof(gsv_t2s_slot_sampling)); }
        hipLaunchKernelGGL(t2s_put_sampling_kernel, dim3(n), dim3(64), 0, S(stream), a);
    }
    HIPCHK(hipGetLastError());
    return GSV_OK;
}

int gsv_t2s_seed_seen(gsv_t2s* h, int batch, const int32_t* slots, const int64_t* tokens, const int32_t* offsets, int nrows, void* stream) {
    if (!h || !h->finalized) return fail(GSV_ERR_STATE, "handle not finalized");
    T2SBound* b = t2s_find(h, batch);
    if (!b) return fail(GSV_ERR_STATE, "no state bound for batch %d", batch);
    if (!slots || !offsets || nrows < 1 || nrows > kAdoptMax || nrows > batch)
        return fail(GSV_ERR_ARG, "seed_seen: need 1..min(batch, %d) rows, their slots and offsets (host arrays)", kAdoptMax);
    for (int i = 0; i < nrows; ++i) {
        if (slots[i] < 0 || slots[i] >= batch) return fail(GSV_ERR_ARG, "seed_seen: slot %d out of range", (int)slots[i]);
        for (int j = 0; j < i; ++j) if (slots[j] == slots[i]) return fail(GSV_ERR_ARG, "seed_seen: slot %d listed twice", (int)slots[i]);
        if (offsets[i] < 0 || offsets[i + 1] < offsets[i]) return fail(GSV_ERR_ARG, "seed_seen: offsets must start at >= 0 and not decrease (row %d)", i);
    }
    if (offsets[nrows] > offsets[0] && !tokens) return fail(GSV_ERR_ARG, "seed_seen: %d tokens listed and no token array", (int)(offsets[nrows] - offsets[0]));
    SeedSeenArgs a;
    a.tokens = tokens; a.seen = (unsigned char*)b->st.seen; a.V = h->cfg.vocab;
    for (int i = 0; i < nrows; ++i) { a.slot[i] = (short)slots[i]; a.off[i] = offsets[i]; }
    a.off[nrows] = offsets[nrows];
    hipLaunchKernelGGL(t2s_seed_seen_kernel, dim3(nrows), dim3(256), 0, S(stream), a);
    HIPCHK(hipGetLastError());
    return GSV_OK;
}

int gsv_t2s_batched_min(gsv_t2s* h) { return h && h->cfg.dtype == GSV_BF16 ? h->batched_min : 0x7fffffff; }
int gsv_t2s_ffn_slices(gsv_t2s* h, int batch) { return !h ? kNJ : ffn_slices(batch); }

size_t gsv_t2s_device_bytes(gsv_t2s* h) {
    if (!h) return 0;
    size_t n = 0;
    for (auto& b : h->arena.blocks) n += b.second;
    return n;
}

int gsv_t2s_set_debug(gsv_t2s* h, void* buf) {
    if (!h) return fail(GSV_ERR_ARG, "null handle");
    h->dbg = (unsigned long long*)buf;
    for (auto& kv : h->bound) t2s_drop_graphs(kv.second);
    return GSV_OK;
}

int gsv_t2s_flush(gsv_t2s* h, int batch, void* stream) {
    if (!h || !h->finalized) return fail(GSV_ERR_STATE, "handle not finalized");
    T2SBound* b = t2s_find(h, batch);
    if (!b) return fail(GSV_ERR_STATE, "no state bound for batch %d", batch);
    return t2s_token(h, b->st, 0, S(stream));
}

}
```

### gsv-tts-lite_amd/csrc/t2s_decode.h

```cpp
#pragma once
#include "gsv_common.h"

namespace gsv {

constexpr int kD = 512;
constexpr int kH = 16;
constexpr int kDh = 32;
constexpr int kF = 2048;
constexpr int kNJ = 32;
constexpr int kFJ = kF / kNJ;
constexpr int kNJFine = 64;
constexpr int kFineMaxB = 4;
inline int ffn_slices(int B) { return B <= kFineMaxB ? kNJFine : kNJ; }
constexpr int kNP = 16;
constexpr float kEps = 1e-5f;

struct TokPart {
    float v;
    int idx;
};

__device__ __forceinline__ void eos_publish(int32_t* eos_host, int slot, int value) {
    if (eos_host != nullptr) __hip_atomic_store(eos_host + slot, value, __ATOMIC_RELAXED, __HIP_MEMORY_SCOPE_SYSTEM);
}


__device__ __forceinline__ void stamp(unsigned long long* dbg, int slot) {
    if (dbg != nullptr && blockIdx.x == 0 && blockIdx.y == 0 && (threadIdx.x == 0 || threadIdx.x == 960))
        dbg[slot < 16 ? slot + (threadIdx.x ? 16 : 0) : 32 + 2 * (slot - 16) + (threadIdx.x ? 1 : 0)] = clock64();
}

constexpr int kNT = 1024;
constexpr int kNW = kNT / 64;

using raw16 = u32x4;

template <typename WT, int N> struct Unpack;
template <> struct Unpack<float, 4> {
    static __device__ __forceinline__ void run(const raw16& r, float (&o)[4]) {
#pragma unroll
        for (int i = 0; i < 4; ++i) o[i] = __uint_as_float(r[i]);
    }
};
template <> struct Unpack<bf16_t, 8> {
    static __device__ __forceinline__ void run(const raw16& r, float (&o)[8]) {
#pragma unroll
        for (int j = 0; j < 4; ++j) {
            o[2 * j] = __uint_as_float(r[j] << 16);
            o[2 * j + 1] = __uint_as_float(r[j] & 0xffff0000u);
        }
    }
};

template <typename WT> struct PartOf { using T = float; };
template <> struct PartOf<bf16_t> { using T = _Float16; };
using f16x8 = __attribute__((ext_vector_type(8))) _Float16;

template <typename WT> struct Geo {
    static constexpr int EPL = 16 / sizeof(WT);
    static constexpr int CPR = kD / EPL / 64;
    using PT = typename PartOf<WT>::T;
};

__device__ __forceinline__ raw16 ldg16(const void* p) { return *reinterpret_cast<const raw16*>(p); }
template <bool NT> __device__ __forceinline__ raw16 ldg16w(const void* p) {
    if constexpr (NT) return __builtin_nontemporal_load(reinterpret_cast<const raw16*>(p)); else return ldg16(p);
}

template <typename WT>
__device__ __forceinline__ float row_dot(const raw16 (&w)[Geo<WT>::CPR], const float (&xr)[8]) {
    constexpr int EPL = Geo<WT>::EPL;
    float a = 0.f;
#pragma unroll
    for (int c = 0; c < Geo<WT>::CPR; ++c) {
        float wv[EPL];
        Unpack<WT, EPL>::run(w[c], wv);
#pragma unroll
        for (int i = 0; i < EPL; ++i) a = fmaf(wv[i], xr[c * EPL + i], a);
    }
    return a;
}
template <typename WT, bool NT = false>
__device__ __forceinline__ void row_load(const WT* row, raw16 (&w)[Geo<WT>::CPR]) {
    const int lane = threadIdx.x & 63;
#pragma unroll
    for (int c = 0; c < Geo<WT>::CPR; ++c) w[c] = ldg16w<NT>(row + c * (kD / Geo<WT>::CPR) + lane * Geo<WT>::EPL);
}
template <typename WT>
__device__ __forceinline__ void lane_x(const float* xs, float (&xr)[8]) {
    const int lane = threadIdx.x & 63;
    constexpr int EPL = Geo<WT>::EPL;
#pragma unroll
    for (int c = 0; c < Geo<WT>::CPR; ++c)
#pragma unroll
        for (int i = 0; i < EPL; ++i) xr[c * EPL + i] = xs[c * (kD / Geo<WT>::CPR) + lane * EPL + i];
}

typedef __bf16 bf16x2_t __attribute__((ext_vector_type(2)));
__device__ __forceinline__ float dot2c(uint32_t w, uint32_t x, float acc) {
    return __builtin_amdgcn_fdot2_f32_bf16(__builtin_bit_cast(bf16x2_t, w), __builtin_bit_cast(bf16x2_t, x), acc, false);
}
__device__ __forceinline__ raw16 x8_load(const uint16_t* __restrict__ v, int first) { return *reinterpret_cast<const raw16*>(v + first); }
__device__ __forceinline__ float dot8(const raw16& w, const raw16& x) {
    float a = 0.f, b = 0.f;
    a = dot2c(w[0], x[0], a); b = dot2c(w[1], x[1], b);
    a = dot2c(w[2], x[2], a); b = dot2c(w[3], x[3], b);
    return a + b;
}
template <bool FAST> __device__ __forceinline__ float sm_exp(float x) {
    if constexpr (FAST) return __builtin_amdgcn_exp2f(x); else return expf(x);
}

template <int N> __device__ __forceinline__ float wave_sumN(const float (&v)[N]);
template <> __device__ __forceinline__ float wave_sumN<8>(const float (&v)[8]) {
    float a[4], b[2];
#pragma unroll
    for (int i = 0; i < 4; ++i) a[i] = halve32_sum(v[i], v[i + 4]);
#pragma unroll
    for (int i = 0; i < 2; ++i) b[i] = halve16_sum(a[i], a[i + 2]);
    return oct_sum(halve8_sum(b[0], b[1]));
}
template <> __device__ __forceinline__ float wave_sumN<4>(const float (&v)[4]) {
    float b[2];
#pragma unroll
    for (int i = 0; i < 2; ++i) b[i] = halve32_sum(v[i], v[i + 2]);
    return row16_sum(halve16_sum(b[0], b[1]));
}
template <> __device__ __forceinline__ float wave_sumN<2>(const float (&v)[2]) {
    return xor16_sum(row16_sum(halve32_sum(v[0], v[1])));
}
template <int N> __device__ __forceinline__ int sumN_index();
template <> __device__ __forceinline__ int sumN_index<2>() { return (threadIdx.x >> 5) & 1; }
template <> __device__ __forceinline__ int sumN_index<8>() {
    const int lane = threadIdx.x & 63;
    return ((lane >> 5) & 1) * 4 + ((lane >> 4) & 1) * 2 + ((lane >> 3) & 1);
}
template <> __device__ __forceinline__ int sumN_index<4>() {
    const int lane = threadIdx.x & 63;
    return ((lane >> 5) & 1) * 2 + ((lane >> 4) & 1);
}

template <bool FAST = false>
__device__ __forceinline__ float ln512(float v, bool owner, float g, float bta, float* red) {
    constexpr int NOW = kD / 64;
    const int w = threadIdx.x >> 6;
    if (!FAST || w < NOW) {
        float s = owner ? v : 0.f, q = s * s;
        s = wave_sum(s);
        q = wave_sum(q);
        if ((threadIdx.x & 63) == 0) { red[2 * w] = s; red[2 * w + 1] = q; }
    }
    __syncthreads();
    if (FAST && w >= NOW) return 0.f;
    float ts = 0.f, tq = 0.f;
#pragma unroll
    for (int i = 0; i < (FAST ? NOW : kNW); ++i) { ts += red[2 * i]; tq += red[2 * i + 1]; }
    const float mean = ts * (1.0f / kD);
    const float var = fmaxf(tq * (1.0f / kD) - mean * mean, 0.f);
    const float rs = FAST ? __builtin_amdgcn_rsqf(var + kEps) : 1.0f / sqrtf(var + kEps);
    return (v - mean) * rs * g + bta;
}

template <int NPART, typename PT = float> struct PartialSum;
template <int NPART> struct PartialSum<NPART, float> {
    static constexpr int NPW = NPART / kNW;
    static_assert(NPART % kNW == 0, "NPART");
    f32x4 p[NPW][2];
    float bias, resid, lng, lnb;
    __device__ __forceinline__ void issue(const float* __restrict__ part, const float* __restrict__ b,
                                          const float* __restrict__ r, const float* __restrict__ g,
                                          const float* __restrict__ beta) {
        const int lane = threadIdx.x & 63, wid = threadIdx.x >> 6;
#pragma unroll
        for (int j = 0; j < NPW; ++j)
#pragma unroll
            for (int c = 0; c < 2; ++c)
                p[j][c] = *reinterpret_cast<const f32x4*>(part + (size_t)(wid * NPW + j) * kD + c * 256 + lane * 4);
        if (threadIdx.x < kD) {
            const int t = threadIdx.x;
            bias = b[t]; resid = r[t]; lng = g[t]; lnb = beta[t];
        }
    }
    __device__ __forceinline__ void park(float* __restrict__ stage) {
        const int lane = threadIdx.x & 63, wid = threadIdx.x >> 6;
#pragma unroll
        for (int c = 0; c < 2; ++c) {
            f32x4 s = p[0][c];
#pragma unroll
            for (int j = 1; j < NPW; ++j) s += p[j][c];
            *reinterpret_cast<f32x4*>(stage + wid * kD + c * 256 + lane * 4) = s;
        }
    }
    __device__ __forceinline__ float finish(const float* __restrict__ stage) {
        const int t = threadIdx.x;
        float s = 0.f;
#pragma unroll
        for (int w = 0; w < kNW; ++w) s += stage[w * kD + t];
        return s + bias + resid;
    }
};

template <int NPART> struct PartialSum<NPART, _Float16> {
    static constexpr int NPW = NPART / kNW;
    static_assert(NPART % kNW == 0, "NPART");
    u32x4 p[NPW][1];
    float bias, resid, lng, lnb;
    __device__ __forceinline__ void issue(const _Float16* __restrict__ part, const float* __restrict__ b,
                                          const float* __restrict__ r, const float* __restrict__ g,
                                          const float* __restrict__ beta) {
        const int lane = threadIdx.x & 63, wid = threadIdx.x >> 6;
#pragma unroll
        for (int j = 0; j < NPW; ++j) p[j][0] = *reinterpret_cast<const u32x4*>(part + (size_t)(wid * NPW + j) * kD + lane * 8);
        if (threadIdx.x < kD) {
            const int t = threadIdx.x;
            bias = b[t]; resid = r[t]; lng = g[t]; lnb = beta[t];
        }
    }
    __device__ __forceinline__ void park(float* __restrict__ stage) {
        const int lane = threadIdx.x & 63, wid = threadIdx.x >> 6;
        float s[8];
#pragma unroll
        for (int j = 0; j < NPW; ++j) {
            const f16x8 h = __builtin_bit_cast(f16x8, p[j][0]);
#pragma unroll
            for (int e = 0; e < 8; ++e) s[e] = j == 0 ? (float)h[e] : s[e] + (float)h[e];
        }
        *reinterpret_cast<f32x4*>(stage + wid * kD + lane * 8) = f32x4{s[0], s[1], s[2], s[3]};
        *reinterpret_cast<f32x4*>(stage + wid * kD + lane * 8 + 4) = f32x4{s[4], s[5], s[6], s[7]};
    }
    __device__ __forceinline__ float finish(const float* __restrict__ stage) {
        const int t = threadIdx.x;
        float s = 0.f;
#pragma unroll
        for (int w = 0; w < kNW; ++w) s += stage[w * kD + t];
        return s + bias + resid;
    }
};

template <int M> __device__ __forceinline__ void argmax_step(float& v, int& idx) {
    const float ov = lane_xor<M>(v);
    const int oi = lane_xor<M>(idx);
    if (ov > v || (ov == v && oi < idx)) { v = ov; idx = oi; }
}

template <int G> __device__ __forceinline__ float group_sum(float v) {
    static_assert(G == 4 || G == 8 || G == 16, "group");
    if constexpr (G == 4) return quad_sum(v);
    else if constexpr (G == 8) return oct_sum(v);
    else return row16_sum(v);
}

template <typename WT, int K> struct Panel {
    static constexpr int EPL = Geo<WT>::EPL;
    static constexpr int LPR = K / EPL;
    static constexpr int RPI = kNT / LPR;
    static constexpr int NIT = kD / RPI;
    raw16 w[NIT];
    template <bool NT = false>
    __device__ __forceinline__ void issue(const WT* __restrict__ panel) {
        const int tid = threadIdx.x;
        const int part = tid % LPR, rsub = tid / LPR;
#pragma unroll
        for (int it = 0; it < NIT; ++it) w[it] = ldg16w<NT>(panel + (size_t)(rsub + it * RPI) * K + part * EPL);
    }
    template <typename OT>
    __device__ __forceinline__ void finish_bf16(const uint16_t* __restrict__ vec_lds, OT* __restrict__ out) {
        static_assert(EPL == 8, "bf16 panels");
        const int tid = threadIdx.x;
        const int part = tid % LPR, rsub = tid / LPR;
        const raw16 x = x8_load(vec_lds, part * 8);
#pragma unroll
        for (int it = 0; it < NIT; ++it) {
            const float s = group_sum<LPR>(dot8(w[it], x));
            if (part == 0) out[rsub + it * RPI] = (OT)s;
        }
    }
    template <typename OT>
    __device__ __forceinline__ void finish(const float* __restrict__ vec_lds, OT* __restrict__ out) {
        const int tid = threadIdx.x;
        const int part = tid % LPR, rsub = tid / LPR;
        float vr[EPL];
#pragma unroll
        for (int i = 0; i < EPL; ++i) vr[i] = vec_lds[part * EPL + i];
#pragma unroll
        for (int it = 0; it < NIT; ++it) {
            float wv[EPL];
            Unpack<WT, EPL>::run(w[it], wv);
            float s = 0.f;
#pragma unroll
            for (int i = 0; i < EPL; ++i) s = fmaf(wv[i], vr[i], s);
            s = group_sum<LPR>(s);
            if (part == 0) out[rsub + it * RPI] = (OT)s;
        }
    }
};


struct StepTok {
    const TokPart* tokpart;
    const int64_t* tok_override;
    const int32_t* ctl;
    const int64_t* x_len;
    int64_t* pre_tokens;
    uint8_t* seen;
    int32_t* step;
    int32_t* eos_at;
    const float* emb;
    const float* pe;
    int V, eos, n_pos;
    int32_t* eos_host;
};
struct StepTokLoads { TokPart tp; int ctl0, ctl2; int64_t ovr, xl; };
__device__ __forceinline__ StepTokLoads steptok_issue(const StepTok& k, int b, int lane) {
    StepTokLoads L;
    L.tp = k.tokpart[(size_t)b * kNP + min(lane, kNP - 1)];
    L.ctl0 = k.ctl[0]; L.ctl2 = k.ctl[2];
    L.ovr = k.tok_override[b];
    L.xl = k.x_len[b];
    return L;
}
__device__ __forceinline__ float steptok_finish(const StepTok& k, const StepTokLoads& L, int b, int lane, int tid, bool owner, int64_t n64,
                                                int T, bool books) {
    float bv = lane < kNP ? L.tp.v : -INFINITY;
    int tok = lane < kNP ? L.tp.idx : 0x7fffffff;
    argmax_step<32>(bv, tok); argmax_step<16>(bv, tok); argmax_step<8>(bv, tok);
    argmax_step<4>(bv, tok); argmax_step<2>(bv, tok); argmax_step<1>(bv, tok);
    if (L.ctl0 != 0) tok = (int)L.ovr;
    if (tok < 0 || tok >= k.V) tok = 0;
    int64_t pos = n64 - L.xl;
    if (pos < 0) pos += k.n_pos;
    if (pos < 0) pos = 0;
    if (pos >= k.n_pos) pos = k.n_pos - 1;
    const float v = owner ? k.emb[(size_t)tok * kD + tid] * 1.0f + k.pe[(size_t)pos * kD + tid] : 0.f;
    if (books) {
        if (n64 >= 0 && n64 <= T) k.pre_tokens[(size_t)b * (T + 1) + n64] = tok;
        if (L.ctl2 != 0 && n64 >= 0) k.seen[(size_t)b * k.V + tok] = 1;
        const int stp = k.step[b];
        if (tok == k.eos && k.eos_at[b] < 0) { k.eos_at[b] = stp; eos_publish(k.eos_host, b, stp); }
        k.step[b] = stp + 1;
    }
    return v;
}

template <typename WT>
struct AttnArgs {
    const float* xdirect;
    const typename PartOf<WT>::T* zpart;
    const float* b2;
    const float* x1;
    const float* ln2g;
    const float* ln2b;
    float* xout;
    const WT* wqkv;
    const float* bqkv;
    const WT* wo;
    WT* kc;
    WT* vc;
    const int64_t* kv_len;
    int T;
    typename PartOf<WT>::T* ypart;
    unsigned long long* dbg;
    StepTok tk;
};

constexpr int kAttnLdsFloats = kD + 96 + 32 + 2 * kNW + kNW * 32 + 2 * kNW + kNW * kD;

template <typename WT, int MODE, int NJ = kNJ, bool NT = false, bool NTKV = false>
__global__ __launch_bounds__(kNT) void t2s_attn_kernel(AttnArgs<WT> a) {
    __shared__ __attribute__((aligned(16))) float smem[kAttnLdsFloats];
    float* xs = smem;
    float* qkv = xs + kD;
    float* att = qkv + 96;
    float* red = att + 32;
    float* pacc = red + 2 * kNW;
    float* pm = pacc + kNW * 32;
    float* pl = pm + kNW;
    float* stage = pl + kNW;
    const int h = blockIdx.x, b = blockIdx.y, tid = threadIdx.x, lane = tid & 63, wid = tid >> 6;
    constexpr int EPL = Geo<WT>::EPL;
    constexpr int CPR = Geo<WT>::CPR;
    constexpr int LPR = kDh / EPL;
    constexpr int AW = sizeof(WT) == 2 ? 8 : kNW;
    constexpr int AW0 = kNW - AW;
    constexpr int RPI = AW * 64 / LPR;
    constexpr int KCH = 2 * kNW / AW;
    const bool aw = (unsigned)(__builtin_amdgcn_readfirstlane(wid) - AW0) < (unsigned)AW;
    constexpr int RW = 96 / kNW;
    const bool owner = tid < kD;
    constexpr bool BF = sizeof(WT) == 2;
    uint16_t* xh = reinterpret_cast<uint16_t*>(xs);
    uint16_t* qh = reinterpret_cast<uint16_t*>(qkv);
    uint16_t* kn = qh + 64;
    uint16_t* atth = reinterpret_cast<uint16_t*>(att);
    stamp(a.dbg, 0);

    int kvl_raw = reinterpret_cast<const int*>(a.kv_len)[2 * b];
    WT* Kp = a.kc + (((size_t)b * kH + h) * a.T) * kDh;
    WT* Vp = a.vc + (((size_t)b * kH + h) * a.T) * kDh;
    const int part = tid % LPR, rsub = tid / LPR - AW0 * 64 / LPR;

    PartialSum<NJ, typename Geo<WT>::PT> ps;
    float xd = 0.f;
    StepTokLoads tl;
    tl.tp.v = 0.f;
    if constexpr (MODE == 0) {
        if (owner) xd = a.xdirect[(size_t)b * kD + tid];
    } else if constexpr (MODE == 2) {
        tl = steptok_issue(a.tk, b, lane);
    } else {
        ps.issue(a.zpart + (size_t)b * NJ * kD, a.b2, a.x1 + (size_t)b * kD, a.ln2g, a.ln2b);
    }
    if constexpr (MODE == 1) __builtin_amdgcn_s_barrier();
    asm volatile("" : : : "memory");
    constexpr bool ROLES = MODE == 1 && AW0 > 0 && NJ == kNJFine;
    const WT* wp = a.wqkv + ((size_t)h * 96 + wid * RW) * kD;
    raw16 wq[RW][CPR];
    float bq;
    const int oi = sumN_index<8>();
    auto issue_wq = [&]() {
#pragma unroll
        for (int r = 0; r < RW; ++r) row_load<WT, NT>(wp + (size_t)r * kD, wq[r]);
        bq = a.bqkv[h * 96 + wid * RW + min(oi, RW - 1)];
    };
    int n, nw;
    auto pin = [&]() {
        stamp(a.dbg, 7);
        if constexpr (MODE == 0) asm volatile("" : "+v"(xd), "+v"(kvl_raw) : : "memory");
        else if constexpr (MODE == 2) asm volatile("" : "+v"(tl.tp.v), "+v"(kvl_raw) : : "memory");
        else asm volatile("" : "+v"(ps.p[0][0]), "+v"(kvl_raw) : : "memory");
        stamp(a.dbg, 1);
        n = kvl_raw;
        nw = n < 0 ? a.T - 1 : (n > a.T - 1 ? a.T - 1 : n);
        if (n > a.T - 1) n = a.T - 1;
        if (n < 0) n = 0;
    };
    if constexpr (!ROLES) {
        issue_wq();
        pin();
    }
    raw16 kreg[KCH], vreg[KCH];
    auto issue_k = [&]() {
        if (AW == kNW || aw) {
#pragma unroll
            for (int it = 0; it < KCH; ++it) kreg[it] = ldg16w<NTKV>(Kp + (size_t)min(rsub + it * RPI, n) * kDh + part * EPL);
        }
    };
    auto issue_v = [&]() {
        if (AW == kNW || aw) {
#pragma unroll
            for (int it = 0; it < KCH; ++it) vreg[it] = ldg16w<NTKV>(Vp + (size_t)min(rsub + it * RPI, n) * kDh + part * EPL);
        }
        asm volatile("" : : : "memory");
    };

    auto qkv_rows = [&]() {
        float acc[8];
        if constexpr (BF) {
            const raw16 x = x8_load(xh, lane * 8);
#pragma unroll
            for (int u = 0; u < 8; ++u) acc[u] = u < RW ? dot8(wq[u < RW ? u : 0][0], x) : 0.f;
        } else {
            float xr[8];
            lane_x<WT>(xs, xr);
#pragma unroll
            for (int u = 0; u < 8; ++u) acc[u] = u < RW ? row_dot<WT>(wq[u < RW ? u : 0], xr) : 0.f;
        }
        const float tot = wave_sumN<8>(acc);
        if ((lane & 7) == 0 && oi < RW) {
            const int row = wid * RW + oi;
            float val = tot + bq;
            WT s = from_f32<WT>(val);
            if (row >= 32) {
                val = to_f32<WT>(s);
                if (row < 64) Kp[(size_t)nw * kDh + row - 32] = s; else Vp[(size_t)nw * kDh + row - 64] = s;
            }
            if constexpr (BF) {
                if (row < 32) qh[row] = f32_to_bf16(val);
                else if (row < 64) kn[row - 32] = s;
                else qkv[row] = val;
            } else {
                qkv[row] = val;
            }
        }
    };

    float v;
    if constexpr (ROLES) {
        if (aw) {
            pin();
            ps.park(stage);
            stamp(a.dbg, 16);
            __syncthreads();
            issue_wq();
            issue_k();
            __syncthreads();
            __syncthreads();
            stamp(a.dbg, 2);
            qkv_rows();
            issue_v();
            asm volatile("; attention waves" : : : "memory");
        } else {
            issue_wq();
            pin();
            ps.park(stage);
            stamp(a.dbg, 16);
            __syncthreads();
            v = ln512<BF>(ps.finish(stage), true, ps.lng, ps.lnb, red);
            xh[tid] = f32_to_bf16(v);
            if (h == 0) a.xout[(size_t)b * kD + tid] = v;
            __syncthreads();
            stamp(a.dbg, 2);
            qkv_rows();
            asm volatile("; owner waves" : : : "memory");
        }
    } else {
        if constexpr (MODE == 0) {
            v = xd;
        } else if constexpr (MODE == 2) {
            v = steptok_finish(a.tk, tl, b, lane, tid, owner, (int64_t)kvl_raw, a.T, h == 0 && tid == 0);
        } else {
            ps.park(stage);
            __syncthreads();
            issue_k();
            if constexpr (AW0 > 0) issue_v();
            v = ln512<BF>(owner ? ps.finish(stage) : 0.f, owner, ps.lng, ps.lnb, red);
            if constexpr (AW0 == 0) issue_v();
        }
        if constexpr (MODE != 1) {
            asm volatile("" : "+v"(v) : : "memory");
            issue_k();
            issue_v();
        }
        if (owner) {
            if constexpr (BF) xh[tid] = f32_to_bf16(v);
            else xs[tid] = v;
            if (h == 0) a.xout[(size_t)b * kD + tid] = v;
        }
        __syncthreads();
        stamp(a.dbg, 2);
        qkv_rows();
    }
    __syncthreads();
    stamp(a.dbg, 3);
    Panel<WT, kDh> po;
    po.template issue<NT>(a.wo + (size_t)h * kD * kDh);

    const float scale = BF ? 0.17677669529663687f * 1.4426950408889634f : 0.17677669529663687f;
    float qr[EPL];
    raw16 qp;
    if constexpr (BF) {
        qp = x8_load(qh, part * 8);
    } else {
#pragma unroll
        for (int i = 0; i < EPL; ++i) qr[i] = qkv[part * EPL + i];
    }
    float m_run = -INFINITY, l_run = 0.f, acc[EPL];
#pragma unroll
    for (int i = 0; i < EPL; ++i) acc[i] = 0.f;
    const int awi = wid - AW0;
    const bool wave0 = __builtin_amdgcn_readfirstlane(wid) == AW0;
    if (AW == kNW || aw) {
    for (int c0 = 0; c0 == 0 || c0 < n; c0 += KCH * RPI) {
        if (c0 > 0) {
#pragma unroll
            for (int it = 0; it < KCH; ++it) {
                kreg[it] = ldg16w<NTKV>(Kp + (size_t)min(c0 + rsub + it * RPI, n) * kDh + part * EPL);
                vreg[it] = ldg16w<NTKV>(Vp + (size_t)min(c0 + rsub + it * RPI, n) * kDh + part * EPL);
            }
        }
        float sv[KCH + 1];
        float cmax = -INFINITY;
#pragma unroll
        for (int it = 0; it < KCH; ++it) {
            const int r = c0 + rsub + it * RPI;
            float s = 0.f;
            if constexpr (BF) {
                s = dot8(kreg[it], qp);
            } else {
                float kk[EPL];
                Unpack<WT, EPL>::run(kreg[it], kk);
#pragma unroll
                for (int i = 0; i < EPL; ++i) s = fmaf(qr[i], kk[i], s);
            }
            s = group_sum<LPR>(s);
            sv[it] = r < n ? s * scale : -INFINITY;
            cmax = max_nn(cmax, sv[it]);
        }
        const bool own = wave0 && c0 == 0;
        sv[KCH] = -INFINITY;
        if (own) {
            float s = 0.f;
            if constexpr (BF) {
                s = dot8(*reinterpret_cast<const raw16*>(kn + part * 8), qp);
            } else {
#pragma unroll
                for (int i = 0; i < EPL; ++i) s = fmaf(qr[i], qkv[32 + part * EPL + i], s);
            }
            s = group_sum<LPR>(s);
            sv[KCH] = tid - AW0 * 64 < LPR ? s * scale : -INFINITY;
            cmax = max_nn(cmax, sv[KCH]);
        }
        cmax = wave_max(cmax);
        const float m_new = max_nn(m_run, cmax);
        const float mref = (m_new == -INFINITY) ? 0.f : m_new;
        const float f = sm_exp<BF>(m_run - mref);
        l_run *= f;
#pragma unroll
        for (int i = 0; i < EPL; ++i) acc[i] *= f;
#pragma unroll
        for (int it = 0; it < KCH; ++it) {
            const float p = sm_exp<BF>(sv[it] - mref);
            const bool live = sv[it] != -INFINITY;
            const raw16 vr = live ? vreg[it] : raw16{0u, 0u, 0u, 0u};
            float vv[EPL];
            Unpack<WT, EPL>::run(vr, vv);
            if (part == 0) l_run += p;
#pragma unroll
            for (int i = 0; i < EPL; ++i) acc[i] = fmaf(p, vv[i], acc[i]);
        }
        if (own) {
            const float p = sm_exp<BF>(sv[KCH] - mref);
            if (part == 0) l_run += p;
#pragma unroll
            for (int i = 0; i < EPL; ++i) acc[i] = fmaf(p, qkv[64 + part * EPL + i], acc[i]);
        }
        m_run = m_new;
    }
    l_run = wave_sum(l_run);
    if constexpr (EPL == 8) {
        float r4[4], r2[2];
#pragma unroll
        for (int i = 0; i < 4; ++i) r4[i] = halve32_sum(acc[i], acc[i + 4]);
#pragma unroll
        for (int i = 0; i < 2; ++i) r2[i] = halve16_sum(r4[i], r4[i + 2]);
        float r1 = halve8_sum(r2[0], r2[1]);
        r1 += lane_xor<4>(r1);
        if ((lane & 4) == 0) pacc[awi * 32 + part * 8 + 4 * (lane >> 5) + 2 * ((lane >> 4) & 1) + ((lane >> 3) & 1)] = r1;
    } else {
        float r2[2];
#pragma unroll
        for (int i = 0; i < 2; ++i) r2[i] = halve32_sum(acc[i], acc[i + 2]);
        float r1 = halve16_sum(r2[0], r2[1]);
        r1 += lane_xor<8>(r1);
        if ((lane & 8) == 0) pacc[awi * 32 + part * 4 + 2 * (lane >> 5) + ((lane >> 4) & 1)] = r1;
    }
    if (lane == 0) { pm[awi] = m_run; pl[awi] = l_run; }
    }
    stamp(a.dbg, 4);
    __syncthreads();
    if (wid == 0) {
        const bool has = (lane & 15) < AW;
        const float mw = has ? pm[lane & 15] : -INFINITY, lw = has ? pl[lane & 15] : 0.f;
        const float M = row16_max(mw);
        const float den = row16_sum(lw * sm_exp<BF>(mw - M));
        const int hf = lane >> 5, d = lane & 31;
        float num = 0.f;
#pragma unroll
        for (int w = 0; w < AW / 2; ++w) num = fmaf(pacc[(hf * (AW / 2) + w) * 32 + d], sm_exp<BF>(pm[hf * (AW / 2) + w] - M), num);
        num = xor32_sum(num);
        if (lane < 32) {
            if constexpr (BF) atth[d] = f32_to_bf16(num * __builtin_amdgcn_rcpf(den));
            else att[d] = num / den;
        }
    }
    __syncthreads();
    stamp(a.dbg, 5);
    if constexpr (BF) po.finish_bf16(atth, a.ypart + ((size_t)b * kH + h) * kD);
    else po.finish(att, a.ypart + ((size_t)b * kH + h) * kD);
    stamp(a.dbg, 6);
}


template <typename WT>
struct FfnArgs {
    const typename PartOf<WT>::T* ypart;
    const float* bo;
    const float* x;
    const float* ln1g;
    const float* ln1b;
    float* x1out;
    const WT* w1;
    const float* b1;
    const WT* w2p;
    typename PartOf<WT>::T* zpart;
    unsigned long long* dbg;
};

template <typename WT, int NJ = kNJ, bool NT = false>
__global__ __launch_bounds__(kNT) void t2s_ffn_kernel(FfnArgs<WT> a) {
    constexpr int FJ = kF / NJ;
    __shared__ __attribute__((aligned(16))) float smem[kD + FJ + 2 * kNW + kNW * kD];
    float* xs = smem;
    float* hb = xs + kD;
    float* red = hb + FJ;
    float* stage = red + 2 * kNW;
    const int j = blockIdx.x, b = blockIdx.y, tid = threadIdx.x, lane = tid & 63, wid = tid >> 6;
    constexpr int CPR = Geo<WT>::CPR;
    constexpr int RW = FJ / kNW;
    const bool owner = tid < kD;
    constexpr bool BF = sizeof(WT) == 2;
    uint16_t* xh = reinterpret_cast<uint16_t*>(xs);
    uint16_t* hbh = reinterpret_cast<uint16_t*>(hb);
    stamp(a.dbg, 8);

    PartialSum<kH, typename Geo<WT>::PT> ps;
    ps.issue(a.ypart + (size_t)b * kH * kD, a.bo, a.x + (size_t)b * kD, a.ln1g, a.ln1b);
    __builtin_amdgcn_s_barrier();
    asm volatile("" : : : "memory");
    const int row0 = j * FJ + wid * RW;
    raw16 w1r[RW][CPR];
#pragma unroll
    for (int r = 0; r < RW; ++r) row_load<WT, NT>(a.w1 + (size_t)(row0 + r) * kD, w1r[r]);
    const int oi = sumN_index<RW>();
    const float b1r = a.b1[row0 + oi];
    asm volatile("" : "+v"(ps.p[0][0]) : : "memory");
    stamp(a.dbg, 9);

    ps.park(stage);
    stamp(a.dbg, 13);
    __syncthreads();
    stamp(a.dbg, 14);
    Panel<WT, FJ> p2;
    p2.template issue<NT>(a.w2p + (size_t)j * kD * FJ);
    asm volatile("" : : : "memory");
    const float v = ln512<BF>(owner ? ps.finish(stage) : 0.f, owner, ps.lng, ps.lnb, red);
    stamp(a.dbg, 15);
    if (owner) {
        if constexpr (BF) xh[tid] = f32_to_bf16(v);
        else xs[tid] = v;
        if (j == 0) a.x1out[(size_t)b * kD + tid] = v;
    }
    __syncthreads();
    stamp(a.dbg, 10);
    {
        float acc[RW];
        if constexpr (BF) {
            const raw16 x = x8_load(xh, lane * 8);
#pragma unroll
            for (int u = 0; u < RW; ++u) acc[u] = dot8(w1r[u][0], x);
        } else {
            float xr[8];
            lane_x<WT>(xs, xr);
#pragma unroll
            for (int u = 0; u < RW; ++u) acc[u] = row_dot<WT>(w1r[u], xr);
        }
        const float tot = wave_sumN<RW>(acc);
        if ((lane & (64 / RW - 1)) == 0) {
            const float hv = fmaxf(tot + b1r, 0.f);
            if constexpr (BF) hbh[wid * RW + oi] = f32_to_bf16(hv);
            else hb[wid * RW + oi] = hv;
        }
    }
    __syncthreads();
    stamp(a.dbg, 11);
    if constexpr (BF) p2.finish_bf16(hbh, a.zpart + ((size_t)b * NJ + j) * kD);
    else p2.finish(hb, a.zpart + ((size_t)b * NJ + j) * kD);
    stamp(a.dbg, 12);
}


constexpr int kSlotSamplingWords = 2;

template <typename WT>
struct LogitsArgs {
    const float* hdirect;
    const typename PartOf<WT>::T* zpart;
    const float* b2;
    const float* x1;
    const float* ln2g;
    const float* ln2b;
    const WT* wp;
    int V, eos;
    int vlimit;
    int slot0;
    const int32_t* slots;
    const int32_t* step;
    const int32_t* ctl;
    const float* fctl;
    const uint8_t* seen;
    float* logits;
    float* hidden;
    TokPart* tokpart;
    int64_t* kv_len;
    int bump;
    const u32x4* tab;
};

template <typename WT, int MODE, int NJ = kNJ, bool TAB = false>
__global__ __launch_bounds__(kNT) void t2s_logits_kernel(LogitsArgs<WT> a) {
    __shared__ __attribute__((aligned(16))) float smem[kD + 2 * kNW + 128 + kNW * kD];
    float* xs = smem;
    float* red = xs + kD;
    float* lg = red + 2 * kNW;
    float* stage = lg + 128;
    const int p = blockIdx.x, r_ = blockIdx.y, tid = threadIdx.x, lane = tid & 63, wid = tid >> 6;
    const int b = a.slots ? a.slots[r_] : a.slot0 + r_;
    constexpr int CPR = Geo<WT>::CPR;
    const int rpb = (a.V + kNP - 1) / kNP;
    const int rww = (rpb + kNW - 1) / kNW;
    const int vbase = p * rpb;
    const int nrow = min(rpb, a.V - vbase);
    const bool owner = tid < kD;

    int c_step = a.step[b], c_sup, c_first, c_rep;
    float c_rp;
    if constexpr (TAB) {
        const u32x4 e1 = a.tab[kSlotSamplingWords * b + 1];
        c_rp = __uint_as_float(e1[2]); c_sup = (int)e1[3]; c_first = 0; c_rep = 0;
    } else {
        c_sup = a.ctl[1]; c_first = a.ctl[7]; c_rep = a.ctl[2];
        c_rp = a.fctl[0];
    }
    PartialSum<NJ, typename Geo<WT>::PT> ps;
    float xd = 0.f;
    if constexpr (MODE == 0) {
        if (owner) xd = a.hdirect[(size_t)r_ * kD + tid];
    } else {
        ps.issue(a.zpart + (size_t)r_ * NJ * kD, a.b2, a.x1 + (size_t)r_ * kD, a.ln2g, a.ln2b);
        __builtin_amdgcn_s_barrier();
    }
    asm volatile("" : : : "memory");
    raw16 wr[8][CPR];
#pragma unroll
    for (int u = 0; u < 8; ++u) {
        const int v = min(vbase + wid * rww + min(u, rww - 1), a.V - 1);
        row_load<WT>(a.wp + (size_t)v * kD, wr[u]);
    }
    const int oi = sumN_index<8>();
    const int myr = wid * rww + oi;
    const uint8_t sn = a.seen[(size_t)b * a.V + min(vbase + myr, a.V - 1)];
    asm volatile("" : "+v"(c_step), "+v"(c_sup), "+v"(c_first), "+v"(c_rep), "+v"(c_rp) : : "memory");
    const bool sup = c_step < c_sup || (a.vlimit < a.V && (TAB ? c_sup > 0 : c_first != 0));
    const bool rep = TAB ? (c_rp != 0.f && c_rp != 1.0f) : c_rep != 0;
    const float rp = c_rp;
    if constexpr (MODE == 0) asm volatile("" : "+v"(xd) : : "memory");
    else asm volatile("" : "+v"(ps.p[0][0]) : : "memory");

    float v;
    if constexpr (MODE == 0) {
        v = xd;
    } else {
        ps.park(stage);
        __syncthreads();
        v = ln512<sizeof(WT) == 2>(owner ? ps.finish(stage) : 0.f, owner, ps.lng, ps.lnb, red);
    }
    if (owner) {
        xs[tid] = v;
        if (p == 0) a.hidden[(size_t)b * kD + tid] = v;
    }
    __syncthreads();
    {
        float xr[8];
        lane_x<WT>(xs, xr);
        float acc[8];
#pragma unroll
        for (int u = 0; u < 8; ++u) acc[u] = row_dot<WT>(wr[u], xr);
        const float tot = wave_sumN<8>(acc);
        if ((lane & 7) == 0 && oi < rww && myr < nrow) {
            const int vv = vbase + myr;
            float l = tot;
            if (vv >= a.vlimit) l = -INFINITY;
            if (sup && (vv == 280 || vv == 486 || vv == a.eos)) l = -INFINITY;
            if (rep && sn) l = l < 0.f ? l * rp : l / rp;
            lg[myr] = l;
            a.logits[(size_t)b * a.V + vv] = l;
        }
    }
    __syncthreads();
    if (wid == 0) {
        float bv = -INFINITY;
        int bi = 0x7fffffff;
        for (int r = lane; r < nrow; r += 64) {
            float l = lg[r];
            if (l > bv || (l == bv && vbase + r < bi)) { bv = l; bi = vbase + r; }
        }
        argmax_step<32>(bv, bi); argmax_step<16>(bv, bi); argmax_step<8>(bv, bi);
        argmax_step<4>(bv, bi); argmax_step<2>(bv, bi); argmax_step<1>(bv, bi);
        if (lane == 0) {
            TokPart tp; tp.v = bv; tp.idx = bi;
            a.tokpart[(size_t)b * kNP + p] = tp;
            if (p == 0 && a.bump) { const int64_t kn = a.kv_len[b]; if (kn >= 0) a.kv_len[b] = kn + 1; }
        }
    }
}


struct TokenArgs {
    const TokPart* tokpart;
    const int64_t* tok_override;
    const int32_t* ctl;
    const int64_t* kv_len;
    const int64_t* x_len;
    int64_t* pre_tokens;
    uint8_t* seen;
    int32_t* step;
    int32_t* eos_at;
    const float* emb;
    const float* pe;
    float* xcur;
    int T, V, eos, n_pos, advance;
    const float* logits;
    const float* fctl;
    int32_t* eos_host;
    const u32x4* tab;
};

__device__ __forceinline__ float t2s_uniform(uint32_t seed_lo, uint32_t seed_hi, uint32_t slot, uint32_t pos, uint32_t step,
                                             uint32_t v) {
    uint32_t h = seed_lo ^ (v * 0x9E3779B1u) ^ (pos * 0x85EBCA77u) ^ (slot * 0xC2B2AE3Du) ^ (step * 0x27D4EB2Fu) ^
                 ((seed_hi << 13) | (seed_hi >> 19));
    h ^= h >> 16; h *= 0x7feb352du; h ^= h >> 15; h *= 0x846ca68bu; h ^= h >> 16;
    h += seed_hi;
    h ^= h >> 16; h *= 0x7feb352du; h ^= h >> 15; h *= 0x846ca68bu; h ^= h >> 16;
    return ((float)(h >> 8) + 0.5f) * (1.0f / 16777216.0f);
}

template <int NPL>
__device__ __forceinline__ int t2s_sample_wave(const float* __restrict__ lg, int V, float temperature, float top_p, int k, uint32_t seed_lo,
                                               uint32_t seed_hi, uint32_t slot, uint32_t pos, uint32_t stp) {
    const int lane = threadIdx.x & 63;
    const float invt = 1.0f / fmaxf(temperature, 1e-5f);
    float x[NPL];
#pragma unroll
    for (int i = 0; i < NPL; ++i) {
        const int v = lane + 64 * i;
        x[i] = v < V ? lg[min(v, V - 1)] * invt : -INFINITY;
    }
    if (top_p > 0.f && top_p < 1.0f) {
        float lmax = -INFINITY; int li = 0x7fffffff;
#pragma unroll
        for (int i = 0; i < NPL; ++i)
            if (x[i] > lmax) { lmax = x[i]; li = lane + 64 * i; }
        argmax_step<32>(lmax, li); argmax_step<16>(lmax, li); argmax_step<8>(lmax, li);
        argmax_step<4>(lmax, li); argmax_step<2>(lmax, li); argmax_step<1>(lmax, li);
        const float lm = lmax * (1.0f / invt);
        float pr[NPL], z = 0.f;
#pragma unroll
        for (int i = 0; i < NPL; ++i) {
            pr[i] = x[i] > -INFINITY ? expf(x[i] * (1.0f / invt) - lm) : 0.f;
            z += pr[i];
        }
        const float iz = 1.0f / wave_sum(z);
#pragma unroll
        for (int i = 0; i < NPL; ++i) pr[i] *= iz;
        unsigned lo = 0u, hi = 0x3f800001u;
        for (int it = 0; it < 31 && hi - lo > 1u; ++it) {
            const unsigned mid = lo + (hi - lo) / 2u;
            const float xm = __uint_as_float(mid);
            float s = 0.f;
#pragma unroll
            for (int i = 0; i < NPL; ++i) s += pr[i] >= xm ? pr[i] : 0.f;
            if (wave_sum(s) <= top_p) hi = mid; else lo = mid;
        }
        const float tau = __uint_as_float(hi);
#pragma unroll
        for (int i = 0; i < NPL; ++i)
            if (!(pr[i] >= tau) && lane + 64 * i != li) x[i] = -INFINITY;
    }
    float pivot = -INFINITY, top = -INFINITY;
    uint32_t removed = 0u;
    const bool compact = k > 0 && k < V && k <= 64;
    float cx = -INFINITY; int cv = 0x7fffffff;
    if (k > 64 && k < V) {
        unsigned key[NPL];
#pragma unroll
        for (int i = 0; i < NPL; ++i) {
            const unsigned b = __float_as_uint(x[i]);
            key[i] = lane + 64 * i < V ? (b ^ ((b >> 31) ? 0xffffffffu : 0x80000000u)) : 0u;
        }
        unsigned lo = 0u, hi = 0xffffffffu;
        for (int it = 0; it < 32; ++it) {
            const unsigned mid = lo + ((hi - lo) >> 1) + ((hi - lo) & 1u);
            int c = 0;
#pragma unroll
            for (int i = 0; i < NPL; ++i) c += (lane + 64 * i < V && key[i] >= mid) ? 1 : 0;
            if ((int)wave_sum((float)c) >= k) lo = mid; else hi = mid - 1u;
            if (lo == hi) break;
        }
        const unsigned pb = lo ^ ((lo >> 31) ? 0x80000000u : 0xffffffffu);
        pivot = __uint_as_float(pb);
        float bv = -INFINITY;
#pragma unroll
        for (int i = 0; i < NPL; ++i) bv = fmaxf(bv, x[i]);
        top = wave_max(bv);
    } else if (k > 0 && k < V) {
        for (int r = 0; r < k; ++r) {
            float bv = -INFINITY; int bs = -1;
#pragma unroll
            for (int i = 0; i < NPL; ++i)
                if (!((removed >> i) & 1u) && lane + 64 * i < V && (bs < 0 || x[i] > bv)) { bv = x[i]; bs = i; }
            const float m = wave_max(bs >= 0 ? bv : -INFINITY);
            const unsigned long long cand = __builtin_amdgcn_ballot_w64(bs >= 0 && bv == m);
            if (cand == 0ull) break;
            const int winner = __builtin_ctzll(cand);
            if (lane == winner) removed |= 1u << bs;
            const int vwin = __builtin_amdgcn_readlane(lane + 64 * bs, winner);
            if (compact && lane == r) { cx = m; cv = vwin; }
            if (r == 0) top = m;
            pivot = m;
        }
    } else {
        float bv = -INFINITY;
#pragma unroll
        for (int i = 0; i < NPL; ++i) bv = fmaxf(bv, x[i]);
        top = wave_max(bv);
    }
    float bv = -INFINITY; int bi = 0x7fffffff;
    uint32_t pend = 0u;
#pragma unroll
    for (int i = 0; i < NPL; ++i) {
        const bool in = lane + 64 * i < V && x[i] > -INFINITY && (compact ? (!((removed >> i) & 1u) && x[i] == pivot) : x[i] >= pivot);
        pend |= in ? 1u << i : 0u;
    }
    bool hc = compact && cx > -INFINITY;
    while (__builtin_amdgcn_ballot_w64(hc || pend != 0u) != 0ull) {
        float tx = cx; int tv = cv;
        bool act = hc;
        if (!hc && pend != 0u) {
#pragma unroll
            for (int i = NPL - 1; i >= 0; --i)
                if ((pend >> i) & 1u) { tx = x[i]; tv = lane + 64 * i; }
            pend &= pend - 1u;
            act = true;
        }
        hc = false;
        if (act) {
            const float u = t2s_uniform(seed_lo, seed_hi, slot, pos, stp, (uint32_t)tv);
            const float sc = (tx - top) - logf(-logf(u));
            if (sc > bv || (sc == bv && tv < bi)) { bv = sc; bi = tv; }
        }
    }
    argmax_step<32>(bv, bi); argmax_step<16>(bv, bi); argmax_step<8>(bv, bi);
    argmax_step<4>(bv, bi); argmax_step<2>(bv, bi); argmax_step<1>(bv, bi);
    return bi < V ? bi : 0;
}

template <bool TAB>
static __global__ __launch_bounds__(256) void t2s_token_kernel(TokenArgs a) {
    __shared__ int s_tok;
    const int b = blockIdx.x, tid = threadIdx.x;
    u32x4 e0 = {}, e1 = {};
    if constexpr (TAB) { e0 = a.tab[kSlotSamplingWords * b]; e1 = a.tab[kSlotSamplingWords * b + 1]; }
    const int ctl0 = a.ctl[0];
    const int mode = TAB && ctl0 != 1 ? (int)e0[0] : ctl0;
    int sampled = -1;
    if (mode == 2 && tid < 64) {
        const float* lg = a.logits + (size_t)b * a.V;
        const uint32_t pos = (uint32_t)a.kv_len[b], stp = (uint32_t)a.step[b];
        const int64_t sid = a.tok_override[b];
        const uint32_t stream = sid > 0 ? (uint32_t)(sid - 1) : (uint32_t)b;
        const float temperature = TAB ? __uint_as_float(e0[2]) : a.fctl[1], top_p = TAB ? __uint_as_float(e0[3]) : a.fctl[2];
        const int k = TAB ? (int)e0[1] : a.ctl[4];
        const uint32_t seed_lo = TAB ? e1[0] : (uint32_t)a.ctl[5], seed_hi = TAB ? e1[1] : (uint32_t)a.ctl[6];
        sampled = a.V <= 64 * 17 ? t2s_sample_wave<17>(lg, a.V, temperature, top_p, k, seed_lo, seed_hi, stream, pos, stp)
                                 : t2s_sample_wave<32>(lg, a.V, temperature, top_p, k, seed_lo, seed_hi, stream, pos, stp);
    }
    if (tid == 0) {
        int tok;
        if (mode == 2) {
            tok = sampled;
        } else if (mode != 0) {
            tok = (int)a.tok_override[b];
        } else {
            float bv = -INFINITY;
            tok = 0x7fffffff;
            for (int p = 0; p < kNP; ++p) {
                TokPart t = a.tokpart[(size_t)b * kNP + p];
                if (t.v > bv || (t.v == bv && t.idx < tok)) { bv = t.v; tok = t.idx; }
            }
        }
        if (tok < 0 || tok >= a.V) tok = 0;
        s_tok = tok;
        const int64_t n = a.kv_len[b];
        if (n >= 0 && n <= a.T) a.pre_tokens[(size_t)b * (a.T + 1) + n] = tok;
        if (a.ctl[2] != 0 && n >= 0) a.seen[(size_t)b * a.V + tok] = 1;
        if (tok == a.eos && a.eos_at[b] < 0) { a.eos_at[b] = a.step[b]; eos_publish(a.eos_host, b, a.step[b]); }
        if (a.advance) a.step[b] += 1;
    }
    __syncthreads();
    const int tok = s_tok;
    int64_t pos = a.kv_len[b] - a.x_len[b];
    if (pos < 0) pos += a.n_pos;
    if (pos < 0) pos = 0;
    if (pos >= a.n_pos) pos = a.n_pos - 1;
    for (int c = tid; c < kD; c += 256)
        a.xcur[(size_t)b * kD + c] = a.emb[(size_t)tok * kD + c] * 1.0f + a.pe[(size_t)pos * kD + c];
}

}
```

Before: 4065 semantic_tokens/s.

## Split logits over more blocks for small batch and bound KV depth in attention

For small batches, the logits projection now uses 64 vocab slices instead of 16, with a fixed per-wave row count. Token partials move to a 64-wide stride padded with neutral entries, and the greedy token reduction becomes a one-wave shuffle argmax. The attention kernel gains a KV-depth template parameter chosen from a tracked upper bound on cache length, so short contexts run fewer K/V chunks. Graphs are cached per depth, which adds host bookkeeping and more captured variants, and the tracked bound must stay correct across adopt, commit and move paths.

```diff
diff --git a/gsv-tts-lite_amd/csrc/gsv_abi.hip b/gsv-tts-lite_amd/csrc/gsv_abi.hip
--- a/gsv-tts-lite_amd/csrc/gsv_abi.hip
+++ b/gsv-tts-lite_amd/csrc/gsv_abi.hip
@@ -136,6 +136,7 @@
 struct T2SStateX : gsv_t2s_state {
     int32_t* eos_host = nullptr;
     u32x4* tab = nullptr;
+    int kd = 4;
 };
 static_assert(sizeof(gsv_t2s_slot_sampling) == sizeof(u32x4) * kSlotSamplingWords, "the token kernel reads an entry as two 16-byte words");
 inline u32x4* tab_of(const gsv_t2s_state& s) { return static_cast<const T2SStateX&>(s).tab; }
@@ -143,10 +144,11 @@
 
 struct T2SBound {
     T2SStateX st;
-    hipGraphExec_t graph = nullptr;
-    hipGraphExec_t graph_ft = nullptr;
     static constexpr int kMaxWin = 8;
-    hipGraphExec_t wgraph[2][kMaxWin + 1] = {};
+    hipGraphExec_t wgraph[3][2][kMaxWin + 1] = {};
+    int kv_bound = 0;
+    int sg_bound = 0;
+    int np_env = 0;
     int64_t *sg_kv = nullptr, *sg_x = nullptr;
     int32_t *sg_step = nullptr, *sg_eos = nullptr;
     float *sg_logits = nullptr, *sg_hidden = nullptr;
@@ -154,11 +156,10 @@
 };
 
 void t2s_drop_graphs(T2SBound& b) {
-    if (b.graph) { (void)hipGraphExecDestroy(b.graph); b.graph = nullptr; }
-    if (b.graph_ft) { (void)hipGraphExecDestroy(b.graph_ft); b.graph_ft = nullptr; }
-    for (auto& row : b.wgraph)
-        for (hipGraphExec_t& g : row)
-            if (g) { (void)hipGraphExecDestroy(g); g = nullptr; }
+    for (auto& depth : b.wgraph)
+        for (auto& row : depth)
+            for (hipGraphExec_t& g : row)
+                if (g) { (void)hipGraphExecDestroy(g); g = nullptr; }
 }
 
 void t2s_free_staging(T2SBound& b) {
@@ -342,6 +343,12 @@
     return GSV_OK;
 }
 
+int tok_fill_neutral(TokPart* dst, int B) {
+    const std::vector<TokPart> init((size_t)B * kTokStride, tok_neutral());
+    HIPCHK(hipMemcpy(dst, init.data(), sizeof(TokPart) * init.size(), hipMemcpyHostToDevice));
+    return GSV_OK;
+}
+
 int t2s_ensure_scratch(gsv_t2s* h, int B) {
     if (B <= h->scratch_b) return GSV_OK;
     for (void* p : {(void*)h->xcur, (void*)h->xbuf, (void*)h->x1buf, (void*)h->ypart, (void*)h->zpart, (void*)h->tokpart})
@@ -351,8 +358,8 @@
     HIPCHK(gsv_dev_malloc(&h->x1buf, sizeof(float) * B * kD));
     HIPCHK(gsv_dev_malloc(&h->ypart, sizeof(float) * B * kH * kD));
     HIPCHK(gsv_dev_malloc(&h->zpart, sizeof(float) * B * kNJFine * kD));
-    HIPCHK(gsv_dev_malloc(&h->tokpart, sizeof(TokPart) * B * kNP));
-    HIPCHK(hipMemset(h->tokpart, 0, sizeof(TokPart) * B * kNP));
+    HIPCHK(gsv_dev_malloc(&h->tokpart, sizeof(TokPart) * B * kTokStride));
+    if (int rc = tok_fill_neutral(h->tokpart, B)) return rc;
     h->scratch_b = B;
     for (auto& kv : h->bound) t2s_drop_graphs(kv.second);
     return GSV_OK;
@@ -397,7 +404,19 @@
             constexpr int MODE = decltype(mode)::value;
             constexpr int NJ = MODE == 1 ? decltype(nj)::value : kNJ;
             constexpr bool NT = MODE == 1 && decltype(nt)::value;
-            hipLaunchKernelGGL((t2s_attn_kernel<WT, MODE, NJ, NT, decltype(ntkv)::value>), dim3(kH, B), dim3(kNT), lds, st, a);
+            auto go = [&](auto kd) {
+                hipLaunchKernelGGL((t2s_attn_kernel<WT, MODE, NJ, NT, decltype(ntkv)::value, decltype(kd)::value>), dim3(kH, B), dim3(kNT), lds, st, a);
+            };
+            if constexpr (sizeof(WT) == 2 && decltype(nj)::value == kNJFine) {
+                const int kd = static_cast<const T2SStateX&>(s).kd;
+                if (kd == 2) go(std::integral_constant<int, 2>{});
+                else if (kd == 3) go(std::integral_constant<int, 3>{});
+                else go(std::integral_constant<int, 4>{});
+            } else if constexpr (sizeof(WT) == 2) {
+                go(std::integral_constant<int, 4>{});
+            } else {
+                go(std::integral_constant<int, 0>{});
+            }
         });
     };
     using Coarse = std::integral_constant<int, kNJ>;
@@ -462,6 +481,11 @@
     return GSV_OK;
 }
 
+inline int logits_slices_env() {
+    const char* e = getenv("GSV_LOGITS_SLICES");
+    return e && atoi(e) == kNP ? kNP : 0;
+}
+
 template <typename WT>
 int t2s_logits(gsv_t2s* h, const gsv_t2s_state& s, int mode, const float* hdirect, int slot0, int nrows, int vlimit,
                int bump, hipStream_t st, const int32_t* slots = nullptr, const T2SBound* staged = nullptr) {
@@ -473,14 +497,24 @@
     a.tokpart = h->tokpart; a.kv_len = s.kv_len; a.bump = bump;
     if (staged) { a.step = staged->sg_step; a.logits = staged->sg_logits; a.hidden = staged->sg_hidden; a.tokpart = staged->sg_tok; a.kv_len = staged->sg_kv; }
     a.tab = tab_of(s);
-    auto launch = [&](auto tab) {
+    const int np = logits_slices_env() == kNP ? kNP : logits_slices(mode == 0 ? nrows : s.batch);
+    const int rww = cdiv(cdiv(h->cfg.vocab, np), kNW);
+    auto launch = [&](auto tab, auto np_c, auto rww_c) {
         constexpr bool TAB = decltype(tab)::value;
-        if (mode == 0) hipLaunchKernelGGL((t2s_logits_kernel<WT, 0, kNJ, TAB>), dim3(kNP, nrows), dim3(kNT), 0, st, a);
-        else if (ffn_slices(s.batch) == kNJFine) hipLaunchKernelGGL((t2s_logits_kernel<WT, 1, kNJFine, TAB>), dim3(kNP, nrows), dim3(kNT), 0, st, a);
-        else hipLaunchKernelGGL((t2s_logits_kernel<WT, 1, kNJ, TAB>), dim3(kNP, nrows), dim3(kNT), 0, st, a);
+        constexpr int NP = decltype(np_c)::value, RWW = decltype(rww_c)::value;
+        if (mode == 0) hipLaunchKernelGGL((t2s_logits_kernel<WT, 0, kNJ, TAB, NP, RWW>), dim3(NP, nrows), dim3(kNT), 0, st, a);
+        else if (ffn_slices(s.batch) == kNJFine) hipLaunchKernelGGL((t2s_logits_kernel<WT, 1, kNJFine, TAB, NP, RWW>), dim3(NP, nrows), dim3(kNT), 0, st, a);
+        else hipLaunchKernelGGL((t2s_logits_kernel<WT, 1, kNJ, TAB, NP, RWW>), dim3(NP, nrows), dim3(kNT), 0, st, a);
     };
-    if (a.tab) launch(std::true_type{});
-    else launch(std::false_type{});
+    auto with_shape = [&](auto tab) {
+        using Any = std::integral_constant<int, 0>;
+        if (np == kNPFine && rww == 2) launch(tab, std::integral_constant<int, kNPFine>{}, std::integral_constant<int, 2>{});
+        else if (np == kNPFine) launch(tab, std::integral_constant<int, kNPFine>{}, Any{});
+        else if (rww == 5) launch(tab, std::integral_constant<int, kNP>{}, std::integral_constant<int, 5>{});
+        else launch(tab, std::integral_constant<int, kNP>{}, Any{});
+    };
+    if (a.tab) with_shape(std::true_type{});
+    else with_shape(std::false_type{});
     HIPCHK(hipGetLastError());
     return GSV_OK;
 }
@@ -705,6 +739,25 @@
     return t2s_logits<WT>(h, s, 1, nullptr, 0, s.batch, h->cfg.vocab, 1, st);
 }
 
+int kv_depth_for(const gsv_t2s* h, const T2SBound& b, int w, bool capturing) {
+    if (h->cfg.dtype != GSV_BF16 || ffn_slices(b.st.batch) != kNJFine || b.st.batch >= h->batched_min) return 4;
+    if (const char* e = getenv("GSV_KV_DEPTH")) {
+        const int f = atoi(e);
+        if (f >= 2 && f <= 4) return f;
+    }
+    if (capturing || b.st.max_kv > 512) return 4;
+    for (int kd = 2; kd < 4; ++kd)
+        if (b.kv_bound + w - 1 <= kd * 128) return kd;
+    return 4;
+}
+bool t2s_capturing(hipStream_t st) {
+    hipStreamCaptureStatus cs = hipStreamCaptureStatusNone;
+    return hipStreamIsCapturing(st, &cs) != hipSuccess || cs != hipStreamCaptureStatusNone;
+}
+void kv_bound_add(T2SBound& b, int n, bool capturing) {
+    b.kv_bound = capturing ? b.st.max_kv : (int)std::min<long long>((long long)b.kv_bound + n, b.st.max_kv);
+}
+
 template <typename WT>
 int t2s_prefill_impl(gsv_t2s* h, T2SBound& bd, int slot0, int nrows, int l_max, float* xy, const int64_t* x_lens,
                      const int64_t* y_lens, void* ws, size_t ws_bytes, hipStream_t st, const int32_t* slots = nullptr, bool staged = false) {
@@ -770,6 +823,9 @@
     if (staged) { fa.kv_len = bd.sg_kv; fa.x_len = bd.sg_x; fa.step = bd.sg_step; fa.eos_at = bd.sg_eos; fa.eos_host = nullptr; }
     hipLaunchKernelGGL(t2s_prefill_finish_kernel, dim3(nrows), dim3(128), 0, st, fa);
     HIPCHK(hipGetLastError());
+    if (staged) bd.sg_bound = std::max(bd.sg_bound, l_max);
+    else if (slots == nullptr && slot0 == 0 && nrows == s.batch) bd.kv_bound = l_max;
+    else bd.kv_bound = std::max(bd.kv_bound, l_max);
     return t2s_logits<WT>(h, s, 0, hlast, slot0, nrows, h->cfg.vocab - 1, 0, st, slots, staged ? &bd : nullptr);
 }
 
@@ -783,7 +839,7 @@
     const int s = a.slots[blockIdx.x], tid = threadIdx.x;
     for (int v = tid; v < a.V; v += 256) a.logits[(size_t)s * a.V + v] = a.sg_logits[(size_t)s * a.V + v];
     for (int c = tid; c < kD; c += 256) a.hidden[(size_t)s * kD + c] = a.sg_hidden[(size_t)s * kD + c];
-    if (tid < kNP) a.tokpart[(size_t)s * kNP + tid] = a.sg_tok[(size_t)s * kNP + tid];
+    if (tid < kTokStride) a.tokpart[(size_t)s * kTokStride + tid] = a.sg_tok[(size_t)s * kTokStride + tid];
     if (tid == 0) { a.kv_len[s] = a.sg_kv[s]; a.x_len[s] = a.sg_x[s]; a.step[s] = a.sg_step[s]; a.eos_at[s] = a.sg_eos[s]; eos_publish(a.eos_host, s, a.sg_eos[s]); }
 }
 
@@ -817,7 +873,7 @@
     const int ss = a.src[blockIdx.x], s = a.dst[blockIdx.x], tid = threadIdx.x;
     for (int v = tid; v < a.V; v += 256) { a.logits[(size_t)s * a.V + v] = a.sg_logits[(size_t)ss * a.V + v]; a.d_seen[(size_t)s * a.V + v] = a.s_seen[(size_t)ss * a.V + v]; }
     for (int c = tid; c < kD; c += 256) a.hidden[(size_t)s * kD + c] = a.sg_hidden[(size_t)ss * kD + c];
-    if (tid < kNP) a.tokpart[(size_t)s * kNP + tid] = a.sg_tok[(size_t)ss * kNP + tid];
+    if (tid < kTokStride) a.tokpart[(size_t)s * kTokStride + tid] = a.sg_tok[(size_t)ss * kTokStride + tid];
     if (tid == 0) {
         a.kv_len[s] = a.sg_kv[ss]; a.x_len[s] = a.sg_x[ss]; a.step[s] = a.sg_step[ss]; a.eos_at[s] = a.sg_eos[ss];
         eos_publish(a.eos_host, s, a.sg_eos[ss]);
@@ -850,10 +906,10 @@
 __global__ __launch_bounds__(256) void t2s_move_state_kernel(MoveArgs a) {
     const int tid = threadIdx.x;
     if (blockIdx.x == a.n) {
-        __shared__ TokPart tp[kAdoptMax * kNP];
-        for (int i = tid; i < a.n * kNP; i += 256) tp[i] = a.tokpart[(size_t)a.src[i / kNP] * kNP + i % kNP];
+        __shared__ TokPart tp[kAdoptMax * kTokStride];
+        for (int i = tid; i < a.n * kTokStride; i += 256) tp[i] = a.tokpart[(size_t)a.src[i / kTokStride] * kTokStride + i % kTokStride];
         __syncthreads();
-        for (int i = tid; i < a.n * kNP; i += 256) a.tokpart[(size_t)a.dst[i / kNP] * kNP + i % kNP] = tp[i];
+        for (int i = tid; i < a.n * kTokStride; i += 256) a.tokpart[(size_t)a.dst[i / kTokStride] * kTokStride + i % kTokStride] = tp[i];
         return;
     }
     const int ss = a.src[blockIdx.x], s = a.dst[blockIdx.x];
@@ -1050,12 +1106,15 @@
     static_cast<gsv_t2s_state&>(b.st) = *st;
     b.st.eos_host = nullptr;
     b.st.tab = nullptr;
+    b.kv_bound = st->max_kv;
+    b.sg_bound = 0;
     t2s_free_staging(b);
     const size_t B = (size_t)st->batch;
     HIPCHK(gsv_dev_malloc(&b.sg_kv, 8 * B)); HIPCHK(gsv_dev_malloc(&b.sg_x, 8 * B));
     HIPCHK(gsv_dev_malloc(&b.sg_step, 4 * B)); HIPCHK(gsv_dev_malloc(&b.sg_eos, 4 * B));
     HIPCHK(gsv_dev_malloc(&b.sg_logits, sizeof(float) * B * h->cfg.vocab)); HIPCHK(gsv_dev_malloc(&b.sg_hidden, sizeof(float) * B * kD));
-    HIPCHK(gsv_dev_malloc(&b.sg_tok, sizeof(TokPart) * B * kNP));
+    HIPCHK(gsv_dev_malloc(&b.sg_tok, sizeof(TokPart) * B * kTokStride));
+    if (int rc = tok_fill_neutral(b.sg_tok, (int)B)) return rc;
     HIPCHK(hipMemset(b.sg_step, 0, 4 * B));
     HIPCHK(hipMemset(b.sg_kv, 0, 8 * B)); HIPCHK(hipMemset(b.sg_x, 0, 8 * B));
     HIPCHK(hipMemset(b.sg_eos, 0xff, 4 * B));
@@ -1152,6 +1211,7 @@
     a.logits = b->st.logits; a.hidden = b->st.hidden; a.tokpart = h->tokpart; a.V = h->cfg.vocab;
     hipLaunchKernelGGL(t2s_commit_kernel, dim3(nrows), dim3(256), 0, S(stream), a);
     HIPCHK(hipGetLastError());
+    b->kv_bound = std::max(b->kv_bound, b->sg_bound);
     return GSV_OK;
 }
 
@@ -1183,6 +1243,7 @@
         hipLaunchKernelGGL(t2s_adopt_state_kernel, dim3(n), dim3(256), 0, S(stream), a);
     }
     HIPCHK(hipGetLastError());
+    d->kv_bound = std::min(d->st.max_kv, std::max(d->kv_bound, sb->sg_bound));
     return GSV_OK;
 }
 
@@ -1215,6 +1276,7 @@
     hipLaunchKernelGGL(t2s_move_kv_kernel, dim3(h->cfg.n_layer * kH, nrows, 2), dim3(256), 0, S(stream), a);
     hipLaunchKernelGGL(t2s_move_state_kernel, dim3(nrows + 1), dim3(256), 0, S(stream), a);
     HIPCHK(hipGetLastError());
+    d->kv_bound = std::min(d->st.max_kv, std::max(d->kv_bound, sb->kv_bound));
     return GSV_OK;
 }
 
@@ -1222,6 +1284,9 @@
     if (!h || !h->finalized) return fail(GSV_ERR_STATE, "handle not finalized");
     T2SBound* b = t2s_find(h, batch);
     if (!b) return fail(GSV_ERR_STATE, "no state bound for batch %d", batch);
+    const bool capturing = t2s_capturing(S(stream));
+    b->st.kd = kv_depth_for(h, *b, 1, capturing);
+    kv_bound_add(*b, 1, capturing);
     if (h->cfg.dtype == GSV_BF16 && batch >= h->batched_min && b->st.max_kv <= 1024) {
         HIPCHK(hipMemcpyAsync(h->xcur, x, sizeof(float) * (size_t)batch * kD, hipMemcpyDeviceToDevice, S(stream)));
         if (int rc = t2s_batched_layers<bf16_t>(h, b->st, S(stream))) return rc;
@@ -1239,15 +1304,25 @@
     if (!b) return fail(GSV_ERR_STATE, "no state bound for batch %d", batch);
     const bool bf = h->cfg.dtype == GSV_BF16;
     const bool graph = (use_graph & 1) != 0, ft = (use_graph & GSV_STEP_FUSED_TOKEN) != 0;
+    const bool capturing = t2s_capturing(S(stream));
+    if (const int ne = logits_slices_env(); ne != b->np_env) {
+        t2s_drop_graphs(*b);
+        b->np_env = ne;
+    }
     if (!graph) {
-        for (int i = 0; i < n_steps; ++i)
+        for (int i = 0; i < n_steps; ++i) {
+            b->st.kd = kv_depth_for(h, *b, 1, capturing);
+            kv_bound_add(*b, 1, capturing);
             if (int rc = bf ? t2s_step<bf16_t>(h, b->st, S(stream), ft) : t2s_step<float>(h, b->st, S(stream), ft)) return rc;
+        }
         return GSV_OK;
     }
     auto graph_of = [&](int steps, hipGraphExec_t** out) -> int {
-        hipGraphExec_t& exec = steps == 1 ? (ft ? b->graph_ft : b->graph) : b->wgraph[ft ? 1 : 0][steps];
+        const int kd = kv_depth_for(h, *b, steps, capturing);
+        hipGraphExec_t& exec = b->wgraph[kd - 2][ft ? 1 : 0][steps];
         *out = &exec;
         if (exec) return GSV_OK;
+        b->st.kd = kd;
         hipGraph_t g = nullptr;
         HIPCHK(hipStreamBeginCapture(h->cap_stream, hipStreamCaptureModeThreadLocal));
         int rc = GSV_OK;
@@ -1267,6 +1342,7 @@
         hipGraphExec_t* exec = nullptr;
         if (int rc = graph_of(w, &exec)) return rc;
         HIPCHK(hipGraphLaunch(*exec, S(stream)));
+        kv_bound_add(*b, w, capturing);
         left -= w;
     }
     return GSV_OK;
@@ -1276,6 +1352,7 @@
     if (!h || !h->finalized || !out_ms || iters < 1) return fail(GSV_ERR_STATE, "bad call");
     T2SBound* b = t2s_find(h, batch);
     if (!b) return fail(GSV_ERR_STATE, "no state bound for batch %d", batch);
+    b->st.kd = kv_depth_for(h, *b, 1, false);
     return h->cfg.dtype == GSV_BF16 ? t2s_time_impl<bf16_t>(h, b, iters, out_ms, S(stream))
                                     : t2s_time_impl<float>(h, b, iters, out_ms, S(stream));
 }
diff --git a/gsv-tts-lite_amd/csrc/t2s_decode.h b/gsv-tts-lite_amd/csrc/t2s_decode.h
--- a/gsv-tts-lite_amd/csrc/t2s_decode.h
+++ b/gsv-tts-lite_amd/csrc/t2s_decode.h
@@ -13,12 +13,17 @@
 constexpr int kFineMaxB = 4;
 inline int ffn_slices(int B) { return B <= kFineMaxB ? kNJFine : kNJ; }
 constexpr int kNP = 16;
+constexpr int kNPFine = 64;
+inline int logits_slices(int rows) { return rows <= kFineMaxB ? kNPFine : kNP; }
+constexpr int kTokStride = 64;
+static_assert(kTokStride == 64 && kNPFine <= kTokStride, "one wave reads a sequence's partials, one per lane");
 constexpr float kEps = 1e-5f;
 
 struct TokPart {
     float v;
     int idx;
 };
+__host__ __device__ inline TokPart tok_neutral() { return TokPart{-INFINITY, 0x7fffffff}; }
 
 __device__ __forceinline__ void eos_publish(int32_t* eos_host, int slot, int value) {
     if (eos_host != nullptr) __hip_atomic_store(eos_host + slot, value, __ATOMIC_RELAXED, __HIP_MEMORY_SCOPE_SYSTEM);
@@ -313,7 +318,7 @@
 struct StepTokLoads { TokPart tp; int ctl0, ctl2; int64_t ovr, xl; };
 __device__ __forceinline__ StepTokLoads steptok_issue(const StepTok& k, int b, int lane) {
     StepTokLoads L;
-    L.tp = k.tokpart[(size_t)b * kNP + min(lane, kNP - 1)];
+    L.tp = k.tokpart[(size_t)b * kTokStride + lane];
     L.ctl0 = k.ctl[0]; L.ctl2 = k.ctl[2];
     L.ovr = k.tok_override[b];
     L.xl = k.x_len[b];
@@ -321,8 +326,8 @@
 }
 __device__ __forceinline__ float steptok_finish(const StepTok& k, const StepTokLoads& L, int b, int lane, int tid, bool owner, int64_t n64,
                                                 int T, bool books) {
-    float bv = lane < kNP ? L.tp.v : -INFINITY;
-    int tok = lane < kNP ? L.tp.idx : 0x7fffffff;
+    float bv = L.tp.v;
+    int tok = L.tp.idx;
     argmax_step<32>(bv, tok); argmax_step<16>(bv, tok); argmax_step<8>(bv, tok);
     argmax_step<4>(bv, tok); argmax_step<2>(bv, tok); argmax_step<1>(bv, tok);
     if (L.ctl0 != 0) tok = (int)L.ovr;
@@ -365,7 +370,7 @@
 
 constexpr int kAttnLdsFloats = kD + 96 + 32 + 2 * kNW + kNW * 32 + 2 * kNW + kNW * kD;
 
-template <typename WT, int MODE, int NJ = kNJ, bool NT = false, bool NTKV = false>
+template <typename WT, int MODE, int NJ = kNJ, bool NT = false, bool NTKV = false, int KD = 0>
 __global__ __launch_bounds__(kNT) void t2s_attn_kernel(AttnArgs<WT> a) {
     __shared__ __attribute__((aligned(16))) float smem[kAttnLdsFloats];
     float* xs = smem;
@@ -383,7 +388,8 @@
     constexpr int AW = sizeof(WT) == 2 ? 8 : kNW;
     constexpr int AW0 = kNW - AW;
     constexpr int RPI = AW * 64 / LPR;
-    constexpr int KCH = 2 * kNW / AW;
+    constexpr int KCH = KD ? KD : 2 * kNW / AW;
+    static_assert(KD == 0 || (sizeof(WT) == 2 && KD >= 2 && KD <= 2 * kNW / AW), "K/V depth: bf16 handles, 2 .. 4");
     const bool aw = (unsigned)(__builtin_amdgcn_readfirstlane(wid) - AW0) < (unsigned)AW;
     constexpr int RW = 96 / kNW;
     const bool owner = tid < kD;
@@ -786,7 +792,7 @@
     const u32x4* tab;
 };
 
-template <typename WT, int MODE, int NJ = kNJ, bool TAB = false>
+template <typename WT, int MODE, int NJ = kNJ, bool TAB = false, int NP = kNP, int RWW = 0>
 __global__ __launch_bounds__(kNT) void t2s_logits_kernel(LogitsArgs<WT> a) {
     __shared__ __attribute__((aligned(16))) float smem[kD + 2 * kNW + 128 + kNW * kD];
     float* xs = smem;
@@ -796,8 +802,9 @@
     const int p = blockIdx.x, r_ = blockIdx.y, tid = threadIdx.x, lane = tid & 63, wid = tid >> 6;
     const int b = a.slots ? a.slots[r_] : a.slot0 + r_;
     constexpr int CPR = Geo<WT>::CPR;
-    const int rpb = (a.V + kNP - 1) / kNP;
-    const int rww = (rpb + kNW - 1) / kNW;
+    const int rpb = (a.V + NP - 1) / NP;
+    const int rww = RWW ? RWW : (rpb + kNW - 1) / kNW;
+    constexpr int NLD = RWW ? RWW : 8;
     const int vbase = p * rpb;
     const int nrow = min(rpb, a.V - vbase);
     const bool owner = tid < kD;
@@ -820,9 +827,9 @@
         __builtin_amdgcn_s_barrier();
     }
     asm volatile("" : : : "memory");
-    raw16 wr[8][CPR];
-#pragma unroll
-    for (int u = 0; u < 8; ++u) {
+    raw16 wr[NLD][CPR];
+#pragma unroll
+    for (int u = 0; u < NLD; ++u) {
         const int v = min(vbase + wid * rww + min(u, rww - 1), a.V - 1);
         row_load<WT>(a.wp + (size_t)v * kD, wr[u]);
     }
@@ -854,7 +861,7 @@
         lane_x<WT>(xs, xr);
         float acc[8];
 #pragma unroll
-        for (int u = 0; u < 8; ++u) acc[u] = row_dot<WT>(wr[u], xr);
+        for (int u = 0; u < 8; ++u) acc[u] = u < NLD ? row_dot<WT>(wr[u < NLD ? u : 0], xr) : 0.f;
         const float tot = wave_sumN<8>(acc);
         if ((lane & 7) == 0 && oi < rww && myr < nrow) {
             const int vv = vbase + myr;
@@ -878,7 +885,10 @@
         argmax_step<4>(bv, bi); argmax_step<2>(bv, bi); argmax_step<1>(bv, bi);
         if (lane == 0) {
             TokPart tp; tp.v = bv; tp.idx = bi;
-            a.tokpart[(size_t)b * kNP + p] = tp;
+            a.tokpart[(size_t)b * kTokStride + p] = tp;
+            if constexpr (NP < kTokStride) {
+                for (int q = p + NP; q < kTokStride; q += NP) a.tokpart[(size_t)b * kTokStride + q] = tok_neutral();
+            }
             if (p == 0 && a.bump) { const int64_t kn = a.kv_len[b]; if (kn >= 0) a.kv_len[b] = kn + 1; }
         }
     }
@@ -1055,6 +1065,14 @@
         sampled = a.V <= 64 * 17 ? t2s_sample_wave<17>(lg, a.V, temperature, top_p, k, seed_lo, seed_hi, stream, pos, stp)
                                  : t2s_sample_wave<32>(lg, a.V, temperature, top_p, k, seed_lo, seed_hi, stream, pos, stp);
     }
+    int greedy = 0x7fffffff;
+    if (mode == 0 && tid < 64) {
+        const TokPart t = a.tokpart[(size_t)b * kTokStride + tid];
+        float bv = t.v;
+        greedy = t.idx;
+        argmax_step<32>(bv, greedy); argmax_step<16>(bv, greedy); argmax_step<8>(bv, greedy);
+        argmax_step<4>(bv, greedy); argmax_step<2>(bv, greedy); argmax_step<1>(bv, greedy);
+    }
     if (tid == 0) {
         int tok;
         if (mode == 2) {
@@ -1062,12 +1080,7 @@
         } else if (mode != 0) {
             tok = (int)a.tok_override[b];
         } else {
-            float bv = -INFINITY;
-            tok = 0x7fffffff;
-            for (int p = 0; p < kNP; ++p) {
-                TokPart t = a.tokpart[(size_t)b * kNP + p];
-                if (t.v > bv || (t.v == bv && t.idx < tok)) { bv = t.v; tok = t.idx; }
-            }
+            tok = greedy;
         }
         if (tok < 0 || tok >= a.V) tok = 0;
         s_tok = tok;
```

Result: no change. 4069 semantic_tokens/s, median of 3 (+0.1%).
